# quziyan/NPairLoss

Measured on NVIDIA H100. Metric: N-pair fwd+bwd samples/sec at B=8192,D=512, higher is better.
Workload: dtype f32 (3-pass fp16-split wgmma, f32 accumulate)

## Files before the change

### npairloss_b200/csrc/ctx.cu

```cuda
#include <cuda.h>
#include <cuda_bf16.h>
#include <cuda_fp16.h>
#include <cuda_runtime.h>
#include <sched.h>
#include <cudaTypedefs.h>
#include <dlfcn.h>

#include <cstdarg>
#include <cstdio>
#include <cstdlib>
#include <cmath>
#include <cstring>
#include <map>
#include <memory>
#include <mutex>
#include <string>
#include <vector>

#include "../../include/npair_b200.h"
#include "gemm_wgmma.cuh"
#include "grad_fused.cuh"
#include "host.cuh"
#include "kernels.cuh"

// ... 14 lines not shown
  fn_ncclGetUniqueId GetUniqueId = nullptr;
  fn_ncclCommInitRank CommInitRank = nullptr;
  fn_ncclCommDestroy CommDestroy = nullptr;
  fn_ncclAllGather AllGather = nullptr;
  fn_ncclReduceScatter ReduceScatter = nullptr;
  fn_ncclGroup GroupStart = nullptr, GroupEnd = nullptr;
  fn_ncclGetErrorString GetErrorString = nullptr;
  std::string err;
};
static NcclApi* nccl_api() {
  static NcclApi api;
  static bool tried = false;
  if (tried) return &api;
  tried = true;
  const char* env = getenv("NPAIR_NCCL_LIB");
  const char* names[] = {env, "libnccl.so.2", "libnccl.so"};
  for (const char* n : names) {
    if (!n) continue;
    api.h = dlopen(n, RTLD_NOW | RTLD_GLOBAL);
    if (api.h) break;
  }
  if (!api.h) { api.err = "libnccl.so.2 not found (set NPAIR_NCCL_LIB)"; return &api; }
#define NPAIR_SYM(name) api.name = reinterpret_cast<decltype(api.name)>(dlsym(api.h, "nccl" #name)); if (!api.name) api.err = "missing symbol nccl" #name;
  NPAIR_SYM(GetUniqueId) NPAIR_SYM(CommInitRank) NPAIR_SYM(CommDestroy) NPAIR_SYM(AllGather) NPAIR_SYM(ReduceScatter)
  NPAIR_SYM(GroupStart) NPAIR_SYM(GroupEnd) NPAIR_SYM(GetErrorString)
#undef NPAIR_SYM
  return &api;
}
enum { NCCL_FLOAT32 = 7, NCCL_SUM = 0 };

struct SharedComm { void* comm; int refs; };
static std::mutex g_comm_mu;
static std::map<std::string, SharedComm> g_comms;
static int acquire_comm(const void* id128, int world, int rank, void** out, std::string* err) {
  NcclApi* api = nccl_api();
  const std::string key(static_cast<const char*>(id128), 128);
  std::lock_guard<std::mutex> lk(g_comm_mu);
  auto it = g_comms.find(key);
  if (it != g_comms.end()) { ++it->second.refs; *out = it->second.comm; return 0; }
  NcclId id; memcpy(&id, id128, 128);
  void* comm = nullptr;
  const int r = api->CommInitRank(&comm, world, id, rank);
  if (r != 0) { *err = fmt("ncclCommInitRank: %s", api->GetErrorString(r)); return r; }
  g_comms[key] = SharedComm{comm, 1};
  *out = comm;
  return 0;
}
static void release_comm(void* comm) {
  NcclApi* api = nccl_api();
  std::lock_guard<std::mutex> lk(g_comm_mu);
  for (auto it = g_comms.begin(); it != g_comms.end(); ++it)
    if (it->second.comm == comm) {
      if (--it->second.refs == 0) { if (api->CommDestroy) api->CommDestroy(comm); g_comms.erase(it); }
      return;
    }
}

static PFN_cuTensorMapEncodeTiled_v12000 tmap_encode_fn() {
  static PFN_cuTensorMapEncodeTiled_v12000 fn = nullptr;
  if (!fn) {
    void* p = nullptr;
    cudaDriverEntryPointQueryResult qres;
    if (cudaGetDriverEntryPoint("cuTensorMapEncodeTiled", &p, cudaEnableDefault, &qres) == cudaSuccess && qres == cudaDriverEntryPointSuccess)
      fn = reinterpret_cast<PFN_cuTensorMapEncodeTiled_v12000>(p);
  }
  return fn;
}

bool make_tmap_pieces(CUtensorMap* m, const void* base, int cols, int rows, int pieces, long long ld_elems,
                      long long piece_stride_elems, int bk, int box_rows, std::string* err) {
  auto fn = tmap_encode_fn();
  if (!fn) { *err = "cuTensorMapEncodeTiled entry point not available"; return false; }
  cuuint64_t dims[3] = {static_cast<cuuint64_t>(cols), static_cast<cuuint64_t>(rows), static_cast<cuuint64_t>(pieces)};
  cuuint64_t strides[2] = {static_cast<cuuint64_t>(ld_elems) * 2ull, static_cast<cuuint64_t>(piece_stride_elems) * 2ull};
  cuuint32_t box[3] = {static_cast<cuuint32_t>(bk), static_cast<cuuint32_t>(box_rows), 1u};
  cuuint32_t estr[3] = {1u, 1u, 1u};
  const CUtensorMapSwizzle sw = (bk * 2 == 128) ? CU_TENSOR_MAP_SWIZZLE_128B : CU_TENSOR_MAP_SWIZZLE_64B;
  CUresult r = fn(m, CU_TENSOR_MAP_DATA_TYPE_UINT16, 3, const_cast<void*>(base), dims, strides, box, estr,
                  CU_TENSOR_MAP_INTERLEAVE_NONE, sw, CU_TENSOR_MAP_L2_PROMOTION_L2_256B, CU_TENSOR_MAP_FLOAT_OOB_FILL_NONE);
  if (r != CUDA_SUCCESS) { *err = fmt("cuTensorMapEncodeTiled failed (%d): cols=%d rows=%d pieces=%d ld=%lld", (int)r, cols, rows, pieces, ld_elems); return false; }
  return true;
}

bool make_tmap_kcat(CUtensorMap* a, CUtensorMap* b, const uint16_t* A, int rows_a, const uint16_t* B, int rows_b, long long kcat,
                    std::string* err) {
  return make_tmap_pieces(a, A, static_cast<int>(kcat), rows_a, 1, kcat, rows_a * kcat, 64, 128, err) &&
         make_tmap_pieces(b, B, static_cast<int>(kcat), rows_b, 1, kcat, rows_b * kcat, 64, 256, err);
}

bool make_tmap_f32_store(CUtensorMap* m, const void* base, int cols, int rows, long long ld_elems, std::string* err, int box_rows) {
  auto fn = tmap_encode_fn();
  if (!fn) { *err = "cuTensorMapEncodeTiled entry point not available"; return false; }
  cuuint64_t dims[2] = {static_cast<cuuint64_t>(cols), static_cast<cuuint64_t>(rows)};
  cuuint64_t strides[1] = {static_cast<cuuint64_t>(ld_elems) * 4ull};
  cuuint32_t box[2] = {32u, static_cast<cuuint32_t>(box_rows)};
  cuuint32_t estr[2] = {1u, 1u};
  CUresult r = fn(m, CU_TENSOR_MAP_DATA_TYPE_FLOAT32, 2, const_cast<void*>(base), dims, strides, box, estr,
                  CU_TENSOR_MAP_INTERLEAVE_NONE, CU_TENSOR_MAP_SWIZZLE_128B, CU_TENSOR_MAP_L2_PROMOTION_NONE, CU_TENSOR_MAP_FLOAT_OOB_FILL_NONE);
  if (r != CUDA_SUCCESS) { *err = fmt("cuTensorMapEncodeTiled(S) failed (%d): cols=%d rows=%d ld=%lld", (int)r, cols, rows, ld_elems); return false; }
  return true;
}

__global__ void p2p_push_kernel(const float* __restrict__ srcA, long long nA, long long offA, const float* __restrict__ srcB, long long nB, long long offB,
                                float* const* __restrict__ peer_base, long long flags_off , int flag_index, int world, uint32_t epoch,
                                unsigned int* ticket) {
  const long long tid = static_cast<long long>(blockIdx.x) * blockDim.x + threadIdx.x, nth = static_cast<long long>(gridDim.x) * blockDim.x;
  const bool vecA = (nA & 3) == 0 && (offA & 3) == 0 && (reinterpret_cast<uintptr_t>(srcA) & 15) == 0;
  if (vecA) {
    for (long long i = tid; i < (nA >> 2); i += nth) {
      const float4 v = reinterpret_cast<const float4*>(srcA)[i];
      for (int r = 0; r < world; ++r) reinterpret_cast<float4*>(peer_base[r] + offA)[i] = v;
    }
  } else {
    for (long long i = tid; i < nA; i += nth) { const float v = srcA[i]; for (int r = 0; r < world; ++r) peer_base[r][offA + i] = v; }
  }
  for (long long i = tid; i < nB; i += nth) { const float v = srcB[i]; for (int r = 0; r < world; ++r) peer_base[r][offB + i] = v; }
  __threadfence_system();
  __syncthreads();
  __shared__ int s_last;
  if (threadIdx.x == 0) s_last = (atomicAdd(ticket, 1u) == gridDim.x - 1) ? 1 : 0;
  __syncthreads();
  if (!s_last) return;
  __threadfence_system();
  if (static_cast<int>(threadIdx.x) < world) {
    uint32_t* f = reinterpret_cast<uint32_t*>(peer_base[threadIdx.x] + flags_off) + flag_index;
    asm volatile("st.release.sys.global.u32 [%0], %1;" ::"l"(f), "r"(epoch) : "memory");
  }
  if (threadIdx.x == 0) *ticket = 0;
}
__global__ void p2p_wait_kernel(const uint32_t* __restrict__ flags , int world, uint32_t epoch) {
  if (static_cast<int>(threadIdx.x) < world) {
    uint32_t v;
    do { asm volatile("ld.acquire.sys.global.u32 %0, [%1];" : "=r"(v) : "l"(flags + threadIdx.x) : "memory"); } while (static_cast<int32_t>(v - epoch) < 0);
  }
}

}

using namespace npair;

#define NPAIR_PROF_PHASES 9
#define NPAIR_INTERNAL_FULL_TILES (1 << 30)
#define NPAIR_XCH_FLOATS 8192
#define NPAIR_H100_SXM_SMS 132

enum { XP_X, XP_LAB, XP_REC, XP_XCH, XP_COUNT };
struct XchgLayout {
  long long base[XP_COUNT], par_stride[XP_COUNT], rank_stride[XP_COUNT], flags, floats;
  long long off(int part, long long par, int rank) const { return base[part] + par * par_stride[part] + rank * rank_stride[part]; }
};
static XchgLayout xchg_layout(int Q, int D, int world, bool world_scope) {
  const long long N = static_cast<long long>(Q) * world;
  const long long rank_floats[XP_COUNT] = {static_cast<long long>(Q) * D, Q, ROW_RECORD_FLOATS * Q, world_scope ? NPAIR_XCH_FLOATS : 0};
  const long long par_floats[XP_COUNT] = {N * D, round_up(N, 4), ROW_RECORD_FLOATS * N, world * rank_floats[XP_XCH]};
  XchgLayout l;
  long long o = 0;
  for (int p = 0; p < XP_COUNT; ++p) { l.base[p] = o; l.par_stride[p] = par_floats[p]; l.rank_stride[p] = rank_floats[p]; o += 2 * par_floats[p]; }
  l.flags = o;
  l.floats = o + round_up(6ll * world, 4);
  return l;
}
static_assert(NPAIR_XCH_FLOATS % 2 == 0, "XCH slots hold 64-bit fields");
enum { XCHG_FEATURES, XCHG_RECORDS, XCHG_SMALL };
static inline int xchg_flag(int kind, int par, int world, int rank) { return (2 * kind + par) * world + rank; }

static int sim_block_rows(const npair_config& c) {
  const long long h = 128ll * ((c.flags >> NPAIR_SIM_BLOCK_SHIFT) & 0xFFF);
  return h < c.Q ? static_cast<int>(h) : 0;
}

static int select_mask(const npair_config& c, int region) {
  return (c.ap_region == region && is_rel(c.ap_method) && !sn_is_max(c.identsn) ? 1 : 0) |
         (c.an_region == region && is_rel(c.an_method) && !sn_is_max(c.diffsn) ? 2 : 0);
}

struct Plan {
  int N, nsplit, bk_grad;
  long long Dp, Np, Qp, ldS;
  long long kcat;
  int bwd_mode;
  bool fused_grad;
  bool cat;
  unsigned int gcand_cap;
  int grad_chunk_kb;
  int grad_kblocks;
  SplitK grad_split;
  int split_cap;
  int n_sym_tiles;
  int s_rows;
  int n_blocks;
  int sweep_epi;
  bool wscope;
  int lsel_mask, gsel_mask;
  bool want_p2p_feat, want_p2p_rec;
  XchgLayout xl;
};

static Plan plan_of(const npair_config& cfg, int sms, bool mma_symmetric, int mem_rows = 0) {
  Plan p{};
  const int prec = cfg.sim_precision, W = cfg.world;
  const long long Q = cfg.Q, D = cfg.D, N = Q * W + mem_rows;
  const bool tc = cfg.gemm_backend == NPAIR_GEMM_TCGEN05, multi = W > 1;
  p.N = static_cast<int>(N);
  p.nsplit = SPLIT_FORMATS[prec].pieces; p.bk_grad = bk_of(prec, EPI_OUT);
  p.Dp = round_up(D, 64); p.Np = round_up(N, 64); p.Qp = round_up(Q, 64); p.ldS = round_up(N, 32);
  p.kcat = mma_passes(p.nsplit) * p.Dp;
  const int blk_rows = sim_block_rows(cfg);
  p.s_rows = blk_rows ? blk_rows : cfg.Q;
  p.n_blocks = (cfg.Q + p.s_rows - 1) / p.s_rows;
  p.wscope = cfg.global_scope && multi;
  p.lsel_mask = select_mask(cfg, NPAIR_LOCAL);
  p.gsel_mask = select_mask(cfg, NPAIR_GLOBAL);
  p.bwd_mode = !multi ? NPAIR_BWDMODE_SINGLE
             : (cfg.bwd_exchange == NPAIR_BWD_AUTO && (!tc || mma_symmetric)) ? NPAIR_BWDMODE_ROW_SCALARS : NPAIR_BWDMODE_REDUCE_SCATTER;
  const bool rs = p.bwd_mode == NPAIR_BWDMODE_REDUCE_SCATTER;
  p.fused_grad = tc && !rs && !(cfg.flags & NPAIR_FLAG_NO_FUSED_GRAD);
  p.cat = tc && prec != PREC_BF16;
  if (p.gsel_mask) {
    const long long cap = Q * N / 8 + 4096;
    p.gcand_cap = static_cast<unsigned int>(cap < (32ll << 20) ? cap : (32ll << 20));
  }
  p.grad_chunk_kb = cfg.grad_chunk_cols > 0 ? (cfg.grad_chunk_cols + 31) / 32 : (cfg.grad_chunk_cols < 0 ? 0 : 64);
  p.grad_kblocks = static_cast<int>(p.fused_grad ? (N + 31) / 32 : (N + p.bk_grad - 1) / p.bk_grad);
  const int tiles = tile_sched(cfg.Q, cfg.D, p.grad_kblocks).num_tiles();
  p.grad_split = tc ? split_k(p.grad_kblocks, tiles, sms, p.fused_grad ? 8 : 4) : SplitK{1, p.grad_kblocks};
  p.split_cap = tc ? split_k_cap(p.grad_kblocks, tiles, sms, p.fused_grad ? 8 : 4) : 1;
  if (!multi && tc && !(cfg.flags & NPAIR_INTERNAL_FULL_TILES) && mem_rows == 0) p.n_sym_tiles = static_cast<int>(sym_tile_count(cfg.Q, p.N));
  p.sweep_epi = EPI_STATS | (p.n_sym_tiles ? EPI_SYM : 0) | (p.n_blocks == 1 ? EPI_STORE_S : 0);
  p.want_p2p_feat = multi && W <= 32 && !(cfg.flags & NPAIR_FLAG_NCCL_FEATURES);
  p.want_p2p_rec = multi && W <= 32 && !(cfg.flags & NPAIR_FLAG_NCCL_RECORDS) && p.bwd_mode == NPAIR_BWDMODE_ROW_SCALARS;
  if (p.want_p2p_feat || p.want_p2p_rec) p.xl = xchg_layout(cfg.Q, cfg.D, W, p.wscope);
  return p;
}

static void carve_rows(Carve& cv, long long Q, long long mem_cap, RowArrays* ra) {
  carve_stats(cv, Q, ra);
  ra->posi_thr = cv.take<float>(Q); ra->nega_thr = cv.take<float>(Q);
  ra->A = cv.take<float>(Q); ra->T = cv.take<float>(Q); ra->logv = cv.take<float>(Q);
  ra->hits = cv.take<int>(3 * Q);
  ra->rowrec = cv.take<RowRecord>(Q + mem_cap, 32);
}

struct npair_ctx : Plan {
  npair_config cfg;
  int Q, D, world, rank, prec, sms, device;
  int mem_cap = 0;
  int mem_rows = 0;
  float* labcat = nullptr;
  DevMem mem;
  float* Xtot_buf = nullptr;
  float* labtot_buf = nullptr;
  float* S = nullptr;
  uint16_t *Xs = nullptr, *XsT = nullptr, *XlT = nullptr, *H = nullptr, *HT = nullptr;
  float* OUT2 = nullptr;
  uint16_t *XcatA = nullptr, *XcatB = nullptr;
  RowRecord* rs_total = nullptr;
  float *Ynorm = nullptr, *dY = nullptr, *inv_norm = nullptr;
  CUtensorMap tm_fB, tm_fS;
  bool p2p_feat = false, p2p_rec = false;
  float* p2p_region = nullptr;
  uint32_t xch_epoch = 0;
  float* xch_src = nullptr;
  float* xch_all = nullptr;
  float** p2p_peer_base = nullptr;
  unsigned int* p2p_ticket = nullptr;
  std::vector<void*> p2p_opened;
  uint32_t p2p_fwd_epoch = 0, p2p_rec_epoch = 0;
  int2* sym_tiles = nullptr;
  int s_block_row0 = -1;
  float* part = nullptr;
  RowArrays ra;
  BlockScalars* bs = nullptr;
  float* partial = nullptr;
  unsigned long long* ghist = nullptr;
  uint32_t* gcand = nullptr;
  TopsBlock* tops_pinned = nullptr;
  unsigned int tops_seq = 0;
  TopsBlock* tops_dev = nullptr;
  AsyncWords* aw = nullptr;
  struct Capture { cudaStream_t st = nullptr; unsigned long long id = 0; } capture;
  CUtensorMap tm_simA, tm_simB, tm_S, tm_b1A, tm_b1B, tm_b2A, tm_b2B;
  void* comm = nullptr; bool own_comm = false;
  struct Step {
    const float* label = nullptr;
    const float *x_total = nullptr, *lab_total = nullptr;
    bool ext_gathered = false;
    bool rec_gathered = false;
    bool fwd_done = false;
    const float *x_mem = nullptr, *lab_mem = nullptr;
  } step;
  StreamOrder order;
  std::string err;
  bool prof = false;
  cudaEvent_t ev[NPAIR_PROF_PHASES + 1][2];
  bool ev_made = false;
  bool ev_used[NPAIR_PROF_PHASES] = {};
};

static cudaError_t ctx_buffers(npair_ctx* c, DevMem& m) {
  const long long Q = c->cfg.Q, D = c->cfg.D, N = c->N;
  const size_t f = sizeof(float), ns = c->nsplit;
  if (c->mem_cap) m.own(&c->labcat, f * N, false);
  if (c->cfg.world > 1) { m.own(&c->Xtot_buf, f * N * D, false); m.own(&c->labtot_buf, f * N, false); }
  if (c->cfg.normalize_input) { m.own(&c->Ynorm, f * Q * D, false); m.own(&c->dY, f * Q * D, false); m.own(&c->inv_norm, f * Q, false); }
  m.own(&c->S, f * c->s_rows * c->ldS, true);
  if (!c->cat) m.own(&c->Xs, 2 * ns * N * c->Dp, true);
  m.own(&c->XsT, 2 * ns * D * c->Np, true);
  if (c->cat) { m.own(&c->XcatA, 2 * Q * c->cfg.world * c->kcat, true); m.own(&c->XcatB, 2 * N * c->kcat, true); }
  if (!c->fused_grad) m.own(&c->H, 2 * ns * Q * c->Np, true);
  if (c->bwd_mode == NPAIR_BWDMODE_REDUCE_SCATTER) { m.own(&c->XlT, 2 * ns * D * c->Qp, true); m.own(&c->HT, 2 * ns * N * c->Qp, true); m.own(&c->OUT2, f * N * D, false); }
  if (c->bwd_mode == NPAIR_BWDMODE_ROW_SCALARS) m.own(&c->rs_total, sizeof(RowRecord) * N, false);
  const int slices = c->mem_cap ? c->split_cap : c->grad_split.splits;
  if (slices > 1) m.own(&c->part, f * split_part(slices, c->cfg.Q, D), false);
  m.own_carved(true, [c](Carve& cv) { carve_rows(cv, c->cfg.Q, c->mem_cap, &c->ra); });
  m.own(&c->bs, sizeof(BlockScalars), true);
  m.own(&c->aw, sizeof(AsyncWords), true);
  m.own(&c->partial, f * 2048, false);
  m.own(&c->ghist, sizeof(unsigned long long) * 4096, true);
  m.own(&c->gcand, sizeof(uint32_t) * 2ull * c->gcand_cap, false);
  m.own(&c->sym_tiles, sizeof(int2) * (c->mem_cap ? sym_tile_count(c->cfg.Q, c->cfg.Q) : c->n_sym_tiles), false);
  if (c->wscope) { m.own(&c->xch_src, f * NPAIR_XCH_FLOATS, false); m.own(&c->xch_all, f * NPAIR_XCH_FLOATS * c->cfg.world, false); }
  return m.err;
}
static cudaError_t p2p_buffers(npair_ctx* c, DevMem& m) {
  m.own(&c->p2p_region, sizeof(float) * c->xl.floats, true);
  m.own(&c->p2p_ticket, sizeof(unsigned int), true);
  m.own(&c->p2p_peer_base, sizeof(float*) * c->cfg.world, false);
  return m.err;
}

struct PhaseTimer {
  npair_ctx* c; int ph; cudaStream_t st;
  PhaseTimer(npair_ctx* c_, int ph_, cudaStream_t st_) : c(c_), ph(ph_), st(st_) {
    if (c->prof) { cudaEventRecord(c->ev[ph][0], st); }
  }
  ~PhaseTimer() {
    if (c->prof) { cudaEventRecord(c->ev[ph][1], st); c->ev_used[ph] = true; }
  }
};

int npair::open_device(int device, int* dev, int* sms) {
  int ndev = 0;
  if (cudaGetDeviceCount(&ndev) != cudaSuccess || ndev < 1) {
    g_create_err = "no CUDA device: libnpair_b200 has no CPU fallback (the oracle under oracle/ is test-only)";
    return NPAIR_E_CUDA;
  }
  if (device >= 0) CREATE_TRY(cudaSetDevice(device));
  CREATE_TRY(cudaGetDevice(dev));
  cudaDeviceProp prop;
  CREATE_TRY(cudaGetDeviceProperties(&prop, *dev));
  if (prop.major != 9 || prop.minor != 0) {
    g_create_err = fmt("device %d is sm_%d%d; this library contains sm_90a code only", *dev, prop.major, prop.minor);
    return NPAIR_E_CUDA;
  }
  *sms = prop.multiProcessorCount;
  return NPAIR_OK;
}

static int validate(const npair_config* c, std::string* err) {
  if (!c) { *err = "null config"; return NPAIR_E_ARG; }
  if (c->Q < 1 || c->D < 1) { *err = "Q and D must be >= 1"; return NPAIR_E_ARG; }
  if (c->world < 1 || c->rank < 0 || c->rank >= c->world) { *err = "bad world/rank"; return NPAIR_E_ARG; }
  if (c->num_tops < 1 || c->num_tops > 5) { *err = "num_tops must be 1..5 (npair_multi_class_loss.hpp:32-34)"; return NPAIR_E_ARG; }
  if (c->ap_region < 0 || c->ap_region > 1 || c->an_region < 0 || c->an_region > 1) { *err = "bad mining region"; return NPAIR_E_ARG; }
  if (c->ap_method < 0 || c->ap_method > 4 || c->an_method < 0 || c->an_method > 4) { *err = "bad mining method"; return NPAIR_E_ARG; }
  if (c->sim_precision < 0 || c->sim_precision > 2) { *err = "bad sim_precision"; return NPAIR_E_ARG; }
  if (c->gemm_backend < 0 || c->gemm_backend > 1) { *err = "bad gemm_backend"; return NPAIR_E_ARG; }
  if (c->bwd_exchange < 0 || c->bwd_exchange > 1) { *err = "bad bwd_exchange"; return NPAIR_E_ARG; }
  if (static_cast<long long>(c->Q) * c->world > 0x7fffffffLL) { *err = "N = Q*world exceeds int32"; return NPAIR_E_ARG; }
  if (c->global_scope < 0 || c->global_scope > 1 || c->normalize_input < 0 || c->normalize_input > 1) { *err = "global_scope / normalize_input must be 0 or 1"; return NPAIR_E_ARG; }
  if (c->grad_chunk_cols > 0 && (c->grad_chunk_cols & 31)) { *err = "grad_chunk_cols must be a multiple of 32"; return NPAIR_E_ARG; }
  if (c->global_scope && c->world > 1 && (c->bwd_exchange != NPAIR_BWD_AUTO || c->gemm_backend != NPAIR_GEMM_TCGEN05 || (c->flags & NPAIR_FLAG_NO_FUSED_GRAD))) {
    *err = "global_scope needs the row-record backward (bwd_exchange AUTO, tensor-core backend, fused gradient kernel)"; return NPAIR_E_ARG;
  }
  if (sim_block_rows(*c)) {
    if (c->gemm_backend != NPAIR_GEMM_TCGEN05 || (c->flags & NPAIR_FLAG_NO_FUSED_GRAD) || c->bwd_exchange != NPAIR_BWD_AUTO) {
      *err = "row-block similarity mode needs the tensor-core backend, the fused gradient kernel and bwd_exchange AUTO"; return NPAIR_E_ARG;
    }
    if (c->global_scope) { *err = "row-block similarity mode does not support global_scope"; return NPAIR_E_ARG; }
    if (select_mask(*c, NPAIR_GLOBAL)) {
      *err = "row-block similarity mode: a GLOBAL RELATIVE_* side needs SN >= 0 with floor(SN) = 0 (its general-SN select sweeps the whole block)";
      return NPAIR_E_ARG;
    }
  }
  return NPAIR_OK;
}

static int validate_memory(const npair_config* c, long long M, std::string* err) {
  if (M < 0) { *err = "max_memory_rows must be >= 0"; return NPAIR_E_ARG; }
  if (M == 0) return NPAIR_OK;
  if (c->world != 1) { *err = "a cross-batch memory needs world = 1"; return NPAIR_E_ARG; }
// ... 22 lines not shown
  std::string e;
  if (validate(cfg, &e) != NPAIR_OK || validate_memory(cfg, max_memory_rows, &e) != NPAIR_OK) return 0;
  npair_ctx c;
  c.cfg = *cfg;
  c.mem_cap = max_memory_rows;
  static_cast<Plan&>(c) = plan_of(*cfg, NPAIR_H100_SXM_SMS, true, max_memory_rows);
  DevMem sizing(false);
  ctx_buffers(&c, sizing);
  if (c.want_p2p_feat || c.want_p2p_rec) p2p_buffers(&c, sizing);
  return sizing.bytes;
}
size_t npair_workspace_bytes(const npair_config* cfg) { return npair_memory_workspace_bytes(cfg, 0); }

const char* npair_last_error(const npair_ctx* ctx) { return ctx ? ctx->err.c_str() : g_create_err.c_str(); }

int npair_nccl_unique_id(void* out) {
  if (!out) return NPAIR_E_ARG;
  NcclApi* api = nccl_api();
  if (!api->h || !api->err.empty()) { g_create_err = api->err; return NPAIR_E_NCCL; }
  NcclId id;
  int r = api->GetUniqueId(&id);
  if (r != 0) { g_create_err = fmt("ncclGetUniqueId: %s", api->GetErrorString(r)); return NPAIR_E_NCCL; }
  memcpy(out, &id, 128);
  return NPAIR_OK;
}

void npair_destroy(npair_ctx* c) {
  if (!c) return;
  if (c->device >= 0) cudaSetDevice(c->device);
  for (void* q : c->p2p_opened) cudaIpcCloseMemHandle(q);
  c->mem.release();
  if (c->comm && c->own_comm) release_comm(c->comm);
  if (c->tops_pinned) cudaFreeHost(c->tops_pinned);
  if (c->ev_made) for (int i = 0; i < NPAIR_PROF_PHASES; ++i) { cudaEventDestroy(c->ev[i][0]); cudaEventDestroy(c->ev[i][1]); }
  delete c;
}

static int create_impl(const npair_config* cfg, const void* id128, void* ext_comm, int mem_cap, npair_ctx** out);
static bool mma_is_symmetric(int prec, int device) {
  static std::mutex mu;
  static std::map<std::pair<int, int>, bool> cache;
  std::lock_guard<std::mutex> lk(mu);
  const std::pair<int, int> key(device, prec);
  auto it = cache.find(key);
  if (it != cache.end()) return it->second;
  bool ok = false;
  const int Q = 192, D = 96;
  npair_config cfg;
  npair_config_default(&cfg, Q, D);
  cfg.sim_precision = prec; cfg.device = device; cfg.flags = NPAIR_INTERNAL_FULL_TILES; cfg.num_tops = 2;
  npair_ctx* t = nullptr;
  if (create_impl(&cfg, nullptr, nullptr, 0, &t) == NPAIR_OK) {
    std::vector<float> x(static_cast<size_t>(Q) * D), lab(Q), S(static_cast<size_t>(Q) * t->ldS);
    uint32_t rng = 12345u;
    for (int r = 0; r < Q; ++r) {
      double nrm = 0.0;
      for (int d = 0; d < D; ++d) { rng = rng * 1664525u + 1013904223u; const float v = static_cast<float>(static_cast<int32_t>(rng >> 8) % 2001 - 1000) * 1e-3f; x[static_cast<size_t>(r) * D + d] = v; nrm += static_cast<double>(v) * v; }
      const float inv = static_cast<float>(1.0 / sqrt(nrm > 0 ? nrm : 1.0));
      for (int d = 0; d < D; ++d) x[static_cast<size_t>(r) * D + d] *= inv;
      lab[r] = static_cast<float>(r / 2);
    }
    float *dx = nullptr, *dl = nullptr;
    float tops[5];
    if (cudaMalloc(&dx, sizeof(float) * x.size()) == cudaSuccess && cudaMalloc(&dl, sizeof(float) * Q) == cudaSuccess &&
        cudaMemcpy(dx, x.data(), sizeof(float) * x.size(), cudaMemcpyHostToDevice) == cudaSuccess &&
        cudaMemcpy(dl, lab.data(), sizeof(float) * Q, cudaMemcpyHostToDevice) == cudaSuccess &&
        npair_forward(t, dx, dl, tops, nullptr) == NPAIR_OK && cudaDeviceSynchronize() == cudaSuccess &&
        cudaMemcpy(S.data(), t->S, sizeof(float) * S.size(), cudaMemcpyDeviceToHost) == cudaSuccess) {
      ok = true;
      for (int i = 0; i < Q && ok; ++i)
        for (int j = 0; j < i; ++j)
          if (memcmp(&S[static_cast<size_t>(i) * t->ldS + j], &S[static_cast<size_t>(j) * t->ldS + i], 4) != 0) { ok = false; break; }
    }
    cudaFree(dx); cudaFree(dl);
    npair_destroy(t);
  }
  cudaGetLastError();
  cache[key] = ok;
  return ok;
}

static bool make_maps(npair_ctx* c, std::string* te) {
  const int Q = c->Q, D = c->D, N = c->N, ns = c->nsplit, bkg = c->bk_grad;
  const uint16_t* catA = c->cat ? c->XcatA : c->Xs;
  const uint16_t* catB = c->cat ? c->XcatB : c->Xs;
  bool ok = make_tmap_kcat(&c->tm_simA, &c->tm_simB, catA +static_cast<long long>(c->rank) * Q * c->kcat, Q, catB, N, c->kcat, te);
  ok = ok && make_tmap_f32_store(&c->tm_S, c->S, N, c->s_rows, c->ldS, te);
  if (c->H) ok = ok && make_tmap_pieces(&c->tm_b1A, c->H, N, Q, ns, c->Np, static_cast<long long>(Q) * c->Np, bkg, 128, te);
  ok = ok && make_tmap_pieces(&c->tm_b1B, c->XsT, N, D, ns, c->Np, static_cast<long long>(D) * c->Np, bkg, 256, te);
  if (c->fused_grad) {
    ok = ok && make_tmap_pieces(&c->tm_fB, c->XsT, N, D, ns, c->Np, static_cast<long long>(D) * c->Np, 32, 256, te);
    ok = ok && make_tmap_f32_store(&c->tm_fS, c->S, N, c->s_rows, c->ldS, te, 128);
  }
  if (c->bwd_mode == NPAIR_BWDMODE_REDUCE_SCATTER) {
    ok = ok && make_tmap_pieces(&c->tm_b2A, c->HT, Q, N, ns, c->Qp, static_cast<long long>(N) * c->Qp, bkg, 128, te);
    ok = ok && make_tmap_pieces(&c->tm_b2B, c->XlT, Q, D, ns, c->Qp, static_cast<long long>(D) * c->Qp, bkg, 256, te);
  }
  return ok;
}

static int set_call_rows(npair_ctx* c, int m) {
  if (!c->mem_cap || m == c->mem_rows) return NPAIR_OK;
  c->step.fwd_done = false;
  const Plan p = plan_of(c->cfg, c->sms, true, m);
  if (p.grad_split.splits > c->split_cap) {
    c->err = fmt("internal: m = %d needs %d split-K slices, the buffer holds %d", m, p.grad_split.splits, c->split_cap);
    return NPAIR_E_STATE;
  }
  c->N = p.N; c->gcand_cap = p.gcand_cap; c->grad_kblocks = p.grad_kblocks; c->grad_split = p.grad_split;
  c->n_sym_tiles = p.n_sym_tiles; c->sweep_epi = p.sweep_epi;
  c->mem_rows = -1;
  std::string te;
  if (!make_maps(c, &te)) { c->err = te; return NPAIR_E_CUDA; }
  c->mem_rows = m;
  return NPAIR_OK;
}

static int create_impl(const npair_config* cfg, const void* id128, void* ext_comm, int mem_cap, npair_ctx** out) {
  if (!out) { g_create_err = "null out"; return NPAIR_E_ARG; }
  *out = nullptr;
  std::string e;
  int rc = validate(cfg, &e);
  if (rc == NPAIR_OK) rc = validate_memory(cfg, mem_cap, &e);
  if (rc != NPAIR_OK) { g_create_err = e; return rc; }
  int device = -1, sms = 0;
  if ((rc = open_device(cfg->device, &device, &sms)) != NPAIR_OK) return rc;
  std::unique_ptr<npair_ctx, void (*)(npair_ctx*)> made(new npair_ctx(), npair_destroy);
  npair_ctx* c = made.get();
  c->cfg = *cfg; c->device = device; c->sms = sms; c->mem_cap = mem_cap; c->mem_rows = mem_cap;
  const bool blocks = sim_block_rows(*cfg) > 0;
  const bool ask_sym = (cfg->world > 1 && cfg->bwd_exchange == NPAIR_BWD_AUTO && cfg->gemm_backend == NPAIR_GEMM_TCGEN05) || blocks;
  const bool sym = !ask_sym || mma_is_symmetric(cfg->sim_precision, c->device);
  if (blocks && !sym) {
    g_create_err = "row-block similarity mode: the similarity GEMM is not bitwise symmetric on this device, so a recomputed block of S "
                   "would not match the rows the statistics were taken from";
    return NPAIR_E_ARG;
  }
  static_cast<Plan&>(*c) = plan_of(*cfg, c->sms, sym, mem_cap);
  c->Q = cfg->Q; c->D = cfg->D; c->world = cfg->world; c->rank = cfg->rank; c->prec = cfg->sim_precision;
  const int Q = c->Q;
  CREATE_TRY(ctx_buffers(c, c->mem));
  if (c->sym_tiles) {
    const std::vector<int2> tl = sym_tile_list(Q, Q);
    CREATE_TRY(cudaMemcpy(c->sym_tiles, tl.data(), sizeof(int2) * tl.size(), cudaMemcpyHostToDevice));
  }
  CREATE_TRY(cudaHostAlloc(&c->tops_pinned, sizeof(TopsBlock), cudaHostAllocMapped));
  memset(c->tops_pinned, 0, sizeof(TopsBlock));
  CREATE_TRY(cudaHostGetDevicePointer(&c->tops_dev, c->tops_pinned, 0));
  CREATE_TRY(c->order.create());
  if (c->lsel_mask) CREATE_TRY(allow_local_select_smem());
  if (cfg->gemm_backend == NPAIR_GEMM_TCGEN05) {
    CREATE_TRY(allow_smem(gemm_kernel(c->prec, c->sweep_epi)));
    if (mem_cap) CREATE_TRY(allow_smem(gemm_kernel(c->prec, plan_of(*cfg, c->sms, sym).sweep_epi)));
    if (c->n_blocks > 1) CREATE_TRY(allow_smem(gemm_kernel(c->prec, EPI_STORE_S)));
    CREATE_TRY(c->fused_grad ? allow_smem(fused_kernel(c->prec)) : allow_smem(gemm_kernel(c->prec, EPI_OUT)));
    std::string te;
    if (!make_maps(c, &te)) { g_create_err = te; return NPAIR_E_CUDA; }
  }
  if (c->world > 1 && (id128 || ext_comm)) {
    NcclApi* api = nccl_api();
    if (!api->h || !api->err.empty()) { g_create_err = api->err; return NPAIR_E_NCCL; }
    if (ext_comm) { c->comm = ext_comm; c->own_comm = false; }
    else {
      std::string ce;
      if (acquire_comm(id128, c->world, c->rank, &c->comm, &ce) != 0) { g_create_err = ce; c->comm = nullptr; return NPAIR_E_NCCL; }
      c->own_comm = true;
    }
  }
  if (c->comm && (c->want_p2p_feat || c->want_p2p_rec) && !getenv("NPAIR_NO_P2P")) {
// ... 190 lines not shown
  if ((rc = async_entry(c, stream, "npair_forward_async", &captured)) != NPAIR_OK) return rc;
  OrderedCall call(c, stream, captured);
  if ((rc = call.enter()) != NPAIR_OK) return rc;
  if ((rc = forward_rank(c, d_feat, d_label, &c->aw->tops, call.st)) != NPAIR_OK) return rc;
  return finish_forward_async(c, d_tops, call.st);
}

int npair_forward_gathered(npair_ctx* c, const float* d_feat_total, const float* d_label_total, float tops_host[5], void* stream) {
  if (!c) return NPAIR_E_ARG;
  if (!d_feat_total || !d_label_total || !tops_host) { c->err = "null pointer argument"; return NPAIR_E_ARG; }
  int rc;
  if ((rc = refuse_capture(c, stream, "npair_forward_gathered")) != NPAIR_OK) return rc;
  OrderedCall call(c, stream);
  if ((rc = call.enter()) != NPAIR_OK) return rc;
  if ((rc = set_call_rows(c, 0)) != NPAIR_OK) return rc;
  const long long r0 = static_cast<long long>(c->rank) * c->Q;
  float* const normed = c->world > 1 ? c->Xtot_buf : c->Ynorm;
  c->step = npair_ctx::Step{d_label_total + r0, c->cfg.normalize_input ? normed : d_feat_total, d_label_total, true};
  if (c->cfg.normalize_input) {
    PhaseTimer pt(c, 1, call.st);
    launch_l2norm_fwd(d_feat_total, c->N, c->D, normed, nullptr, call.st);
    launch_l2norm_fwd(d_feat_total + r0 * c->D, c->Q, c->D, c->Ynorm, c->inv_norm, call.st);
  }
  if ((rc = forward_impl(c, c->step.x_total + r0 * c->D, c->tops_dev, call.st)) != NPAIR_OK) return rc;
  return finish_forward(c, tops_host, call.st);
}

static int memory_call_args(npair_ctx* c, int m) {
  const int rc = validate_memory(&c->cfg, 1, &c->err);
  if (rc != NPAIR_OK) return rc;
  if (m < 0 || m > c->mem_cap) { c->err = fmt("m = %d memory rows outside [0, %d] (npair_create_memory)", m, c->mem_cap); return NPAIR_E_ARG; }
  return NPAIR_OK;
}
static int forward_memory_rows(npair_ctx* c, const float* d_feat, const float* d_label, const float* d_mem_feat, const float* d_mem_label, int m,
                               TopsBlock* tops, cudaStream_t st) {
  const int rc = set_call_rows(c, m);
  if (rc != NPAIR_OK) return rc;
  c->step = npair_ctx::Step{d_label, nullptr, c->labcat};
  c->step.x_mem = d_mem_feat; c->step.lab_mem = d_mem_label;
  if (c->cfg.normalize_input) {
    PhaseTimer pt(c, 1, st);
    launch_l2norm_fwd(d_feat, c->Q, c->D, c->Ynorm, c->inv_norm, st);
    d_feat = c->Ynorm;
  }
  c->step.x_total = d_feat;
  return forward_impl(c, d_feat, tops, st);
}

int npair_forward_memory(npair_ctx* c, const float* d_feat, const float* d_label, const float* d_mem_feat, const float* d_mem_label, int32_t m,
                         float tops_host[5], void* stream) {
  if (!c) return NPAIR_E_ARG;
  if (!d_feat || !d_label || !tops_host || (m > 0 && (!d_mem_feat || !d_mem_label))) { c->err = "null pointer argument"; return NPAIR_E_ARG; }
  int rc;
  if ((rc = memory_call_args(c, m)) != NPAIR_OK) return rc;
  if (m == 0) return npair_forward(c, d_feat, d_label, tops_host, stream);
  if ((rc = refuse_capture(c, stream, "npair_forward_memory")) != NPAIR_OK) return rc;
  OrderedCall call(c, stream);
  if ((rc = call.enter()) != NPAIR_OK) return rc;
  if ((rc = forward_memory_rows(c, d_feat, d_label, d_mem_feat, d_mem_label, m, c->tops_dev, call.st)) != NPAIR_OK) return rc;
  return finish_forward(c, tops_host, call.st);
}

int npair_forward_memory_async(npair_ctx* c, const float* d_feat, const float* d_label, const float* d_mem_feat, const float* d_mem_label,
                               int32_t m, float* d_tops, void* stream) {
  if (!c) return NPAIR_E_ARG;
  if (!d_feat || !d_label || !d_tops || (m > 0 && (!d_mem_feat || !d_mem_label))) { c->err = "null pointer argument"; return NPAIR_E_ARG; }
  int rc;
  if ((rc = memory_call_args(c, m)) != NPAIR_OK) return rc;
  if (m == 0) return npair_forward_async(c, d_feat, d_label, d_tops, stream);
  bool captured = false;
  if ((rc = async_entry(c, stream, "npair_forward_memory_async", &captured)) != NPAIR_OK) return rc;
  OrderedCall call(c, stream, captured);
  if ((rc = call.enter()) != NPAIR_OK) return rc;
  if ((rc = forward_memory_rows(c, d_feat, d_label, d_mem_feat, d_mem_label, m, &c->aw->tops, call.st)) != NPAIR_OK) return rc;
  return finish_forward_async(c, d_tops, call.st);
}

static SimRows sim_rows(const npair_ctx* c, int r0, int rows) {
  return SimRows{c->S, c->ldS, c->Q, c->N, r0, rows, c->step.label, c->step.lab_total, c->rank * c->Q};
}

static cudaError_t sim_gemm(npair_ctx* c, int epi, int r0, int rows, cudaStream_t st) {
  const SimRows sim = sim_rows(c, r0, rows);
  GemmParams gp = sim_sweep(epi, rows, c->N, c->kcat, &c->bs->x_inv_scale, c->sym_tiles, c->n_sym_tiles, c->ra);
  gp.a_row0 = sim.row0; gp.S = c->S; gp.ldS = sim.ldS;
  if (epi & EPI_STATS) {
    gp.lab_rows = sim.lab_rows; gp.lab_cols = sim.lab_cols; gp.self_offset = sim.col0;
    gp.fuse_thr = 1; gp.ra = c->ra; gp.mp = mining_of(c->cfg); gp.bs = c->bs;
    gp.thr_out = c->wscope ? reinterpret_cast<BlockStats*>(c->xch_src) : nullptr;
  }
  return launch_gemm(c->prec, epi, c->tm_simA, c->tm_simB, c->tm_S, gp, c->sms, st);
}

static cudaError_t recompute_sim_block(npair_ctx* c, int r0, cudaStream_t st) {
  if (c->s_block_row0 == r0) return cudaSuccess;
  const cudaError_t e = sim_gemm(c, EPI_STORE_S, r0, c->Q - r0 < c->s_rows ? c->Q - r0 : c->s_rows, st);
  c->s_block_row0 = e == cudaSuccess ? r0 : -1;
  return e;
}

static int forward_impl(npair_ctx* c, const float* d_feat, TopsBlock* tops, cudaStream_t st) {
  const int Q = c->Q, N = c->N, D = c->D;
  const MiningParams mp = mining_of(c->cfg);
  const int self_off = c->rank * Q;
  const bool lsel_warp = (c->cfg.flags & NPAIR_FLAG_LSEL_WARP) != 0;
  {
    PhaseTimer pt(c, 1, st);
    if (c->step.x_mem) {
      const int m = N - Q;
      launch_memory_rows(c->step.label, Q, c->step.lab_mem, m, c->labcat, c->ra.rowrec, st);
      launch_prep_reduce_memory(d_feat, static_cast<long long>(Q) * D, c->step.x_mem, static_cast<long long>(m) * D, c->partial,
                                c->prec == PREC_FP16X2 ? 1 : 0, c->ra, Q, c->bs, st);
      launch_split_memory(d_feat, Q, c->step.x_mem, N, D, c->prec, c->bs, c->Xs, c->Dp, c->XsT, c->Np, c->XcatA, c->XcatB, c->Dp, st);
    } else {
      launch_prep_reduce(d_feat, static_cast<long long>(Q) * D, c->step.x_total, static_cast<long long>(N) * D, c->partial,
                         c->prec == PREC_FP16X2 ? 1 : 0, c->ra, Q, c->bs, st);
      launch_split(c->step.x_total, N, D, c->prec, c->bs, c->Xs, c->Dp, c->XsT, c->Np, c->XlT, c->Qp, self_off, Q, c->XcatA, c->XcatB, c->Dp, st);
    }
  }
  c->s_block_row0 = c->n_blocks == 1 ? 0 : -1;
  if (c->cfg.gemm_backend == NPAIR_GEMM_TCGEN05) {
    PhaseTimer pt(c, 2, st);
    CUDA_TRY(c, sim_gemm(c, c->sweep_epi, 0, Q, st));
  } else {
    GemmParams gp; memset(&gp, 0, sizeof(gp));
    gp.M = Q; gp.Nn = N; gp.S = c->S; gp.ldS = c->ldS; gp.dev_scale = &c->bs->x_inv_scale;
    CUDA_TRY(c, launch_simt_gemm(c->prec, EPI_STORE_S, c->Xs + static_cast<long long>(self_off) * c->Dp, c->Dp, static_cast<long long>(N) * c->Dp,
                                 c->Xs, c->Dp, static_cast<long long>(N) * c->Dp, D, gp, st));
    launch_row_stats_ref(sim_rows(c, 0, Q), c->ra, st);
  }
  {
    PhaseTimer pt(c, 3, st);
    if (c->cfg.gemm_backend != NPAIR_GEMM_TCGEN05) launch_thresholds(c->ra, Q, N, mp, c->bs, st);
    if (c->wscope) {
      const float* all = nullptr;
      const int rc = xchg_small(c, c->xch_src, sizeof(BlockStats) / sizeof(float), &all, st);
      if (rc != NPAIR_OK) return rc;
      launch_thresholds_world(all, NPAIR_XCH_FLOATS, c->world, N, mp, c->bs, st);
    }
    if (c->gsel_mask) {
      for (int pass = 0; pass < 3; ++pass) {
        launch_global_select_pass(sim_rows(c, 0, Q), c->gsel_mask, pass, c->ra, c->ghist, c->gcand, c->gcand_cap, c->wscope ? 1 : 0, c->bs, c->sms,
                                  st);
        if (c->wscope) {
          const float* all = nullptr;
          const int rc = xchg_small(c, reinterpret_cast<const float*>(c->ghist), NPAIR_XCH_FLOATS, &all, st);
          if (rc != NPAIR_OK) return rc;
          launch_global_decide(all, NPAIR_XCH_FLOATS, c->world, c->gsel_mask, pass, c->ra, Q, c->ghist, c->gcand, c->gcand_cap, c->bs, st);
        }
      }
    }
    if (c->lsel_mask && c->n_blocks == 1)
      launch_local_select(sim_rows(c, 0, Q), c->lsel_mask, c->cfg.identsn, c->cfg.diffsn, c->ra, c->bs, c->sms, lsel_warp, st);
  }
  {
    PhaseTimer pt(c, 4, st);
    ++c->tops_seq;
    for (int r0 = 0; r0 < Q; r0 += c->s_rows) {
      const int rows = Q - r0 < c->s_rows ? Q - r0 : c->s_rows;
      CUDA_TRY(c, recompute_sim_block(c, r0, st));
      const SimRows sim = sim_rows(c, r0, rows);
      if (c->lsel_mask && c->n_blocks > 1)
        launch_local_select(sim, c->lsel_mask, c->cfg.identsn, c->cfg.diffsn, c->ra, c->bs, c->sms, lsel_warp, st);
      launch_lse_rows(sim, mp, c->ra, c->bs, c->cfg.num_tops, tops, c->world, c->wscope ? reinterpret_cast<TopSums*>(c->xch_src) : nullptr,
                      weight_scale_log2(c->prec), c->tops_seq, c->n_blocks == 1, st);
    }
    if (c->n_blocks > 1) launch_lse_finalize(Q, N, c->ra, c->bs, c->cfg.num_tops, tops, c->tops_seq, st);
// ... 405 lines not shown
```

### npairloss_b200/csrc/device.cuh

```cuda
#pragma once
#include <cuda_bf16.h>
#include <cuda_fp16.h>
#include <cfloat>

#include "kernels.cuh"

namespace npair {

__device__ __forceinline__ float warp_sum(float v) {
#pragma unroll
  for (int o = 16; o > 0; o >>= 1) v += __shfl_xor_sync(0xffffffffu, v, o);
  return v;
}
__device__ __forceinline__ int warp_sum_i(int v) {
#pragma unroll
  for (int o = 16; o > 0; o >>= 1) v += __shfl_xor_sync(0xffffffffu, v, o);
  return v;
}
__device__ __forceinline__ float warp_max(float v) {
#pragma unroll
  for (int o = 16; o > 0; o >>= 1) v = fmaxf(v, __shfl_xor_sync(0xffffffffu, v, o));
  return v;
}
__device__ __forceinline__ float warp_min(float v) {
#pragma unroll
  for (int o = 16; o > 0; o >>= 1) v = fminf(v, __shfl_xor_sync(0xffffffffu, v, o));
  return v;
}

template <int PREC>
__device__ __forceinline__ void split3(float v, uint16_t& p0, uint16_t& p1, uint16_t& p2) {
  if (PREC == PREC_BF16) {
    p0 = __bfloat16_as_ushort(__float2bfloat16_rn(v)); p1 = 0; p2 = 0;
  } else if (PREC == PREC_FP16X2) {
    const __half h = __float2half_rn(v);
    const float r = v - __half2float(h);
    p0 = __half_as_ushort(h); p1 = __half_as_ushort(__float2half_rn(r)); p2 = 0;
  } else {
    const __nv_bfloat16 h = __float2bfloat16_rn(v);
    const float r1 = v - __bfloat162float(h);
    const __nv_bfloat16 m = __float2bfloat16_rn(r1);
    const float r2 = r1 - __bfloat162float(m);
    p0 = __bfloat16_as_ushort(h); p1 = __bfloat16_as_ushort(m); p2 = __bfloat16_as_ushort(__float2bfloat16_rn(r2));
  }
}
template <int PREC>
__device__ __forceinline__ void split8(const float (&v)[8], float sc, uint16_t (&p)[8][3], uint4 (&pk)[3]) {
#pragma unroll
  for (int e = 0; e < 8; ++e) split3<PREC>(v[e] * sc, p[e][0], p[e][1], p[e][2]);
#pragma unroll
  for (int s = 0; s < SPLIT_FORMATS[PREC].pieces; ++s)
    pk[s] = make_uint4(p[0][s] | (static_cast<uint32_t>(p[1][s]) << 16), p[2][s] | (static_cast<uint32_t>(p[3][s]) << 16),
                       p[4][s] | (static_cast<uint32_t>(p[5][s]) << 16), p[6][s] | (static_cast<uint32_t>(p[7][s]) << 16));
}
template <int PREC>
__device__ __forceinline__ void store_kcat_row(uint16_t* row, long long Dp, int d, const uint4 (&pk)[3], bool side_b) {
  *reinterpret_cast<uint4*>(row + d) = pk[0];
  if (PREC == PREC_FP16X2) {
    *reinterpret_cast<uint4*>(row + Dp + 2 * d) = side_b ? pk[1] : pk[0];
    *reinterpret_cast<uint4*>(row + Dp + 2 * d + 8) = side_b ? pk[0] : pk[1];
  } else if (PREC == PREC_BF16X3) {
    *reinterpret_cast<uint4*>(row + Dp + d) = pk[1];
    *reinterpret_cast<uint4*>(row + 2 * Dp + 2 * d) = side_b ? pk[1] : pk[0];
    *reinterpret_cast<uint4*>(row + 2 * Dp + 2 * d + 8) = side_b ? pk[0] : pk[1];
    *reinterpret_cast<uint4*>(row + 4 * Dp + 2 * d) = side_b ? pk[2] : pk[0];
    *reinterpret_cast<uint4*>(row + 4 * Dp + 2 * d + 8) = side_b ? pk[0] : pk[2];
  }
}

__device__ __forceinline__ void reset_row_stats(const RowArrays& ra, long long i) {
  ra.st_minw[i] = f2ord(FLT_MAX); ra.st_maxw[i] = f2ord(-FLT_MAX);
  ra.st_maxb[i] = f2ord(-FLT_MAX); ra.st_maxall[i] = f2ord(-FLT_MAX);
  ra.cnt_same[i] = 0;
}

}
```

### npairloss_b200/csrc/eval.cu

```cuda
#include <cuda_runtime.h>

#include <cmath>
#include <cstdint>
#include <memory>
#include <string>
#include <vector>

#include "../../include/npair_b200.h"
#include "gemm_wgmma.cuh"
#include "host.cuh"
#include "kernels.cuh"

using namespace npair;

static constexpr int EVAL_NO_SELF = -(1 << 30);

struct EvalPlan {
  int max_q, max_g, D, prec;
  long long Dp, kcat;
  int n_sym_tiles;
};

static int eval_validate(long long max_q, long long max_g, long long D, int prec, std::string* err) {
  if (max_q < 1 || max_g < 1 || D < 1) { *err = "max_queries, max_gallery and D must be >= 1"; return NPAIR_E_ARG; }
  if (max_q >= (1 << 30) || max_g >= (1 << 30) || D >= (1 << 24)) { *err = "max_queries and max_gallery must be < 2^30, D < 2^24"; return NPAIR_E_ARG; }
  if (prec < 0 || prec > 2) { *err = "bad precision"; return NPAIR_E_ARG; }
  return NPAIR_OK;
}

static EvalPlan eval_plan_of(int max_q, int max_g, int D, int prec) {
  EvalPlan p{};
  p.max_q = max_q; p.max_g = max_g; p.D = D; p.prec = prec;
  p.Dp = round_up(D, 64);
  p.kcat = mma_passes(SPLIT_FORMATS[prec].pieces) * p.Dp;
  const int n = max_q < max_g ? max_q : max_g;
  p.n_sym_tiles = static_cast<int>(sym_tile_count(n, n));
  return p;
}

struct npair_eval : EvalPlan {
  int device = -1, sms = 0;
  DevMem mem;
  uint16_t *catA = nullptr, *catB = nullptr;
  RowArrays ra{};
  unsigned int* absmax_bits = nullptr;
  BlockScalars* bs = nullptr;
  int2* sym_tiles = nullptr;
  int sym_n = 0;
  std::vector<int2> sym_host;
  DevMem map_rows_mem, map_pairs_mem, km_mem, knn_mem, cb_mem;
  char *map_rows = nullptr, *map_pairs = nullptr, *km = nullptr, *knn = nullptr, *cb = nullptr;
  StreamOrder order;
  std::string err;
};

static cudaError_t eval_buffers(npair_eval* ev, DevMem& m) {
  m.own(&ev->catA, 2ull * ev->max_q * ev->kcat, false);
  m.own(&ev->catB, 2ull * ev->max_g * ev->kcat, false);
  m.own_carved(true, [ev](Carve& cv) { carve_stats(cv, ev->max_q, &ev->ra); ev->absmax_bits = cv.take<unsigned int>(1); });
  m.own(&ev->bs, sizeof(BlockScalars), true);
  m.own(&ev->sym_tiles, sizeof(int2) * ev->n_sym_tiles, false);
  return m.err;
}

struct MapRows : Carve {
  long long* seg; unsigned long long* sum_err; int* fill;
  MapRows(char* base, long long nq) : Carve{base} { seg = take<long long>(nq + 1); sum_err = take<unsigned long long>(2); fill = take<int>(nq); }
};
struct MapPairs : Carve {
  float* pos; unsigned int* hist;
  MapPairs(char* base, long long sum_r) : Carve{base} { pos = take<float>(sum_r); hist = take<unsigned int>(sum_r); }
};
struct KmeansBufs : Carve {
  long long* sums; unsigned long long* keys; double* partial; int* counts; float* bias; int* rows; KmeansWords* words;
  KmeansBufs(char* base, long long n, long long k, long long D) : Carve{base} {
    sums = take<long long>(k * D); keys = take<unsigned long long>(n); partial = take<double>(KM_INERTIA_BLOCKS);
    counts = take<int>(k); bias = take<float>(k); rows = take<int>(k); words = take<KmeansWords>(1);
  }
};
struct KnnBlock : Carve {
  float* S; long long ldS;
  KnnBlock(char* base, long long rows, long long ng) : Carve{base}, ldS(round_up(ng, 32)) { S = take<float>(rows * ldS); }
};
static_assert(KNN_MAX_K == NPAIR_EVAL_KNN_MAX_K, "the select's capacity is the call's limit on k");
static constexpr int KNN_DEFAULT_BLOCK_ROWS = 1024;
static int knn_block_rows(int block_rows, int nq) {
  const long long rows = block_rows ? block_rows : KNN_DEFAULT_BLOCK_ROWS, cap = round_up(nq, 128);
  return static_cast<int>(rows < cap ? rows : cap);
}
struct ClassBatchBufs : Carve {
  float* S; long long ldS; int* pools;
  ClassBatchBufs(char* base, long long C, long long pool_size, long long n_batches) : Carve{base}, ldS(round_up(C, 32)) {
    S = take<float>(C * ldS); pools = take<int>(n_batches * pool_size);
  }
};
static_assert(CLASS_POOL_MAX == NPAIR_EVAL_CLASS_POOL_MAX, "the greedy kernel's capacity is the call's limit on the pool size");

static int eval_grow(npair_eval* ev, DevMem& m, char** base, size_t bytes, const char* what) {
  if (bytes <= m.bytes) return NPAIR_OK;
  m.release();
  m.own(base, bytes, false);
  if (m.err == cudaSuccess) return NPAIR_OK;
  cudaGetLastError();
  m.release();
  ev->err = fmt("cannot allocate %zu bytes for %s", bytes, what);
  return NPAIR_E_CUDA;
}

extern "C" {

size_t npair_eval_workspace_bytes(int32_t max_q, int32_t max_g, int32_t D, int32_t prec) {
  std::string e;
  if (eval_validate(max_q, max_g, D, prec, &e) != NPAIR_OK) return 0;
  npair_eval ev;
  static_cast<EvalPlan&>(ev) = eval_plan_of(max_q, max_g, D, prec);
  DevMem sizing(false);
  eval_buffers(&ev, sizing);
  return sizing.bytes;
}

size_t npair_eval_map_at_r_bytes(int32_t nq, int64_t sum_r) {
  if (nq < 1 || sum_r < 0) return 0;
  return MapRows(nullptr, nq).bytes + MapPairs(nullptr, sum_r).bytes;
}

size_t npair_eval_kmeans_bytes(int32_t n, int32_t k, int32_t D) {
  if (n < 1 || k < 1 || D < 1 || k > n) return 0;
  return KmeansBufs(nullptr, n, k, D).bytes;
}

size_t npair_eval_knn_bytes(int32_t ng, int32_t k, int32_t block_rows) {
  if (ng < 1 || k < 1 || k > NPAIR_EVAL_KNN_MAX_K || k > ng || block_rows < 0 || block_rows % 128) return 0;
  return KnnBlock(nullptr, block_rows ? block_rows : KNN_DEFAULT_BLOCK_ROWS, ng).bytes;
}

size_t npair_eval_class_batches_bytes(int32_t n_classes, int32_t pool_size, int32_t n_batches) {
  if (n_classes < 1 || n_batches < 1 || pool_size < 2 || pool_size > n_classes || pool_size > NPAIR_EVAL_CLASS_POOL_MAX) return 0;
  return ClassBatchBufs(nullptr, n_classes, pool_size, n_batches).bytes;
}

const char* npair_eval_last_error(const npair_eval* ev) { return ev ? ev->err.c_str() : g_create_err.c_str(); }

void npair_eval_destroy(npair_eval* ev) {
  if (!ev) return;
  if (ev->device >= 0) cudaSetDevice(ev->device);
  delete ev;
}

int npair_eval_create(int32_t max_q, int32_t max_g, int32_t D, int32_t prec, int32_t device, npair_eval** out) {
  if (!out) { g_create_err = "null out"; return NPAIR_E_ARG; }
  *out = nullptr;
  int rc = eval_validate(max_q, max_g, D, prec, &g_create_err);
  if (rc != NPAIR_OK) return rc;
  int dev = -1, sms = 0;
  if ((rc = open_device(device, &dev, &sms)) != NPAIR_OK) return rc;
  std::unique_ptr<npair_eval, void (*)(npair_eval*)> made(new npair_eval(), npair_eval_destroy);
  npair_eval* ev = made.get();
  static_cast<EvalPlan&>(*ev) = eval_plan_of(max_q, max_g, D, prec);
  ev->device = dev; ev->sms = sms;
  CREATE_TRY(eval_buffers(ev, ev->mem));
  CREATE_TRY(ev->order.create());
  const int epis[] = {EPI_STATS, EPI_STATS | EPI_SYM, EPI_COUNT, EPI_COUNT | EPI_SYM, EPI_GATHER, EPI_GATHER | EPI_SYM, EPI_BUCKET,
                      EPI_BUCKET | EPI_SYM, EPI_ARGMAX, EPI_STORE_S};
  for (int epi : epis) CREATE_TRY(allow_smem(gemm_kernel(prec, epi)));
  CREATE_TRY(allow_knn_select_smem());
  *out = made.release();
  return NPAIR_OK;
}

}

static int eval_check(npair_eval* ev, const float* q, int nq, const float* g, int ng, int self_offset, int gallery_row0, float absmax,
                      bool whole_gallery) {
  if (!q || !g) { ev->err = "null pointer argument"; return NPAIR_E_ARG; }
  if (nq < 1 || ng < 1) { ev->err = "nq and ng must be >= 1"; return NPAIR_E_ARG; }
  if (nq > ev->max_q || ng > ev->max_g) { ev->err = fmt("nq = %d, ng = %d exceed the evaluator's capacity (%d, %d)", nq, ng, ev->max_q, ev->max_g); return NPAIR_E_ARG; }
  if (self_offset < -1) { ev->err = "self_offset must be -1 (disjoint sets) or >= 0"; return NPAIR_E_ARG; }
  if (whole_gallery && self_offset >= 0 && static_cast<long long>(self_offset) + nq > ng) { ev->err = "self_offset + nq exceeds ng"; return NPAIR_E_ARG; }
  if (gallery_row0 < 0) { ev->err = "gallery_row0 must be >= 0"; return NPAIR_E_ARG; }
  if (!(absmax >= 0.f) && !whole_gallery) { ev->err = "absmax must be max|x| over the queries and the whole gallery (>= 0)"; return NPAIR_E_ARG; }
  if (!std::isfinite(absmax) && !whole_gallery) { ev->err = "absmax must be finite"; return NPAIR_E_ARG; }
  return NPAIR_OK;
}

static int eval_self_col(int self_offset, int gallery_row0) { return self_offset < 0 ? EVAL_NO_SELF : self_offset - gallery_row0; }
static bool eval_sym(const float* q, int nq, const float* g, int ng, int self_col) { return q == g && nq == ng && self_col == 0; }

static int eval_prepare(npair_eval* ev, const float* q, int nq, const float* g, int ng, float absmax, bool sym, cudaStream_t st) {
  const long long D = ev->D;
  unsigned int* amx = nullptr;
  if (absmax < 0.f && ev->prec == PREC_FP16X2) {
    amx = ev->absmax_bits;
    CUDA_TRY(ev, cudaMemsetAsync(amx, 0, sizeof(unsigned int), st));
  }
  launch_eval_prep(q, nq * D, sym ? nullptr : g, ng * D, amx, ev->ra, nq, ev->sms, st);
  launch_eval_split(q, nq, ev->D, ev->Dp, ev->prec, 0, absmax, amx, ev->bs, ev->catA, st);
  launch_eval_split(g, ng, ev->D, ev->Dp, ev->prec, 1, absmax, amx, ev->bs, ev->catB, st);
  CUDA_TRY(ev, cudaGetLastError());
  return NPAIR_OK;
}

static int eval_sweep(npair_eval* ev, int epi, int nq, int ng, int self_col, const float* ql, const float* gl, const float* cut, int32_t* count,
                      bool sym, cudaStream_t st, const GemmParams* map = nullptr) {
  if (sym) {
    if (ev->sym_n != nq) {
      ev->sym_host = sym_tile_list(nq, nq);
      CUDA_TRY(ev, cudaMemcpyAsync(ev->sym_tiles, ev->sym_host.data(), sizeof(int2) * ev->sym_host.size(), cudaMemcpyHostToDevice, st));
      ev->sym_n = nq;
    }
    epi |= EPI_SYM;
  }
  GemmParams gp = sim_sweep(epi, nq, ng, ev->kcat, &ev->bs->x_inv_scale, ev->sym_tiles, static_cast<int>(ev->sym_host.size()), ev->ra);
  gp.self_offset = self_col;
  if (epi & (EPI_STATS | EPI_GATHER | EPI_BUCKET)) { gp.lab_rows = ql; gp.lab_cols = gl; }
  else { gp.cut = cut; gp.count = count; }
  if (map) {
    gp.cnt_same = ev->ra.cnt_same; gp.bs = ev->bs; gp.seg = map->seg; gp.fill = map->fill; gp.pos = map->pos; gp.hist = map->hist;
    gp.col_bias = map->col_bias; gp.best = map->best;
  }
  CUtensorMap ta, tb;
  std::string te;
  if (!make_tmap_kcat(&ta, &tb, ev->catA, nq, ev->catB, ng, ev->kcat, &te)) { ev->err = te; return NPAIR_E_CUDA; }
  CUDA_TRY(ev, launch_gemm(ev->prec, epi, ta, tb, ta, gp, ev->sms, st));
  return NPAIR_OK;
}

extern "C" {

int npair_eval_rank(npair_eval* ev, const float* q, const float* ql, int32_t nq, const float* g, const float* gl, int32_t ng, int32_t self_offset,
                    int32_t* d_rank, void* stream) {
  if (!ev) return NPAIR_E_ARG;
  int rc = eval_check(ev, q, nq, g, ng, self_offset, 0, -1.f, true);
  if (rc != NPAIR_OK) return rc;
  if (!ql || !gl || !d_rank) { ev->err = "null pointer argument"; return NPAIR_E_ARG; }
  OrderedCall call(ev, stream);
  if ((rc = call.enter()) != NPAIR_OK) return rc;
  const cudaStream_t st = call.st;
  const int self_col = eval_self_col(self_offset, 0);
  const bool sym = eval_sym(q, nq, g, ng, self_col);
  float* cut = reinterpret_cast<float*>(ev->ra.st_minw);
  if ((rc = eval_prepare(ev, q, nq, g, ng, -1.f, sym, st)) != NPAIR_OK) return rc;
  if ((rc = eval_sweep(ev, EPI_STATS, nq, ng, self_col, ql, gl, nullptr, nullptr, sym, st)) != NPAIR_OK) return rc;
  launch_eval_best(ev->ra, nq, cut, st);
  CUDA_TRY(ev, cudaMemsetAsync(d_rank, 0, sizeof(int32_t) * nq, st));
  if ((rc = eval_sweep(ev, EPI_COUNT, nq, ng, self_col, nullptr, nullptr, cut, d_rank, sym, st)) != NPAIR_OK) return rc;
  CUDA_TRY(ev, cudaGetLastError());
  return NPAIR_OK;
}

int npair_eval_best_positive(npair_eval* ev, const float* q, const float* ql, int32_t nq, const float* g, const float* gl, int32_t ng,
                             int32_t self_offset, int32_t gallery_row0, float absmax, float* d_best, void* stream) {
  if (!ev) return NPAIR_E_ARG;
  int rc = eval_check(ev, q, nq, g, ng, self_offset, gallery_row0, absmax, false);
  if (rc != NPAIR_OK) return rc;
  if (!ql || !gl || !d_best) { ev->err = "null pointer argument"; return NPAIR_E_ARG; }
  OrderedCall call(ev, stream);
  if ((rc = call.enter()) != NPAIR_OK) return rc;
  const cudaStream_t st = call.st;
  const int self_col = eval_self_col(self_offset, gallery_row0);
  const bool sym = eval_sym(q, nq, g, ng, self_col);
  if ((rc = eval_prepare(ev, q, nq, g, ng, absmax, sym, st)) != NPAIR_OK) return rc;
  if ((rc = eval_sweep(ev, EPI_STATS, nq, ng, self_col, ql, gl, nullptr, nullptr, sym, st)) != NPAIR_OK) return rc;
  launch_eval_best(ev->ra, nq, d_best, st);
  CUDA_TRY(ev, cudaGetLastError());
  return NPAIR_OK;
}

int npair_eval_count(npair_eval* ev, const float* q, int32_t nq, const float* g, int32_t ng, int32_t self_offset, int32_t gallery_row0,
                     float absmax, const float* d_cut, int32_t* d_count, void* stream) {
  if (!ev) return NPAIR_E_ARG;
  int rc = eval_check(ev, q, nq, g, ng, self_offset, gallery_row0, absmax, false);
  if (rc != NPAIR_OK) return rc;
  if (!d_cut || !d_count) { ev->err = "null pointer argument"; return NPAIR_E_ARG; }
  OrderedCall call(ev, stream);
  if ((rc = call.enter()) != NPAIR_OK) return rc;
  const cudaStream_t st = call.st;
  const int self_col = eval_self_col(self_offset, gallery_row0);
  const bool sym = eval_sym(q, nq, g, ng, self_col);
  if ((rc = eval_prepare(ev, q, nq, g, ng, absmax, sym, st)) != NPAIR_OK) return rc;
  CUDA_TRY(ev, cudaMemsetAsync(d_count, 0, sizeof(int32_t) * nq, st));
  if ((rc = eval_sweep(ev, EPI_COUNT, nq, ng, self_col, nullptr, nullptr, d_cut, d_count, sym, st)) != NPAIR_OK) return rc;
  CUDA_TRY(ev, cudaGetLastError());
  return NPAIR_OK;
}

int npair_eval_knn(npair_eval* ev, const float* q, int32_t nq, const float* g, int32_t ng, int32_t self_offset, int32_t gallery_row0,
                   float absmax, int32_t k, int32_t block_rows, float* d_sim, int32_t* d_index, void* stream) {
  if (!ev) return NPAIR_E_ARG;
  int rc = eval_check(ev, q, nq, g, ng, self_offset, gallery_row0, absmax < 0.f ? 0.f : absmax, false);
  if (rc != NPAIR_OK) return rc;
  if (!d_sim || !d_index) { ev->err = "null pointer argument"; return NPAIR_E_ARG; }
  if (static_cast<long long>(gallery_row0) + ng > INT32_MAX) { ev->err = "gallery_row0 + ng exceeds the int32 index range"; return NPAIR_E_ARG; }
  if (block_rows < 0 || block_rows % 128) { ev->err = fmt("block_rows = %d must be 0 or a positive multiple of 128", block_rows); return NPAIR_E_ARG; }
  long long self_col = self_offset < 0 ? EVAL_NO_SELF : static_cast<long long>(self_offset) - gallery_row0;
  if (self_col >= ng || self_col + nq <= 0) self_col = EVAL_NO_SELF;
  const int valid = self_col == EVAL_NO_SELF ? ng : ng - 1;
  if (k < 1 || k > NPAIR_EVAL_KNN_MAX_K || k > valid) {
    ev->err = fmt("k = %d must lie in [1, %d] and not exceed the %d candidate columns of a query", k, NPAIR_EVAL_KNN_MAX_K, valid);
    return NPAIR_E_ARG;
  }
  OrderedCall call(ev, stream);
  if ((rc = call.enter()) != NPAIR_OK) return rc;
  const cudaStream_t st = call.st;
  const int rows = knn_block_rows(block_rows, nq);
  if ((rc = eval_grow(ev, ev->knn_mem, &ev->knn, KnnBlock(nullptr, rows, ng).bytes, "the k-NN block of S")) != NPAIR_OK) return rc;
  const KnnBlock blk(ev->knn, rows, ng);
  if ((rc = eval_prepare(ev, q, nq, g, ng, absmax, false, st)) != NPAIR_OK) return rc;
  CUtensorMap ta, tb;
  std::string te;
  if (!make_tmap_kcat(&ta, &tb, ev->catA, nq, ev->catB, ng, ev->kcat, &te)) { ev->err = te; return NPAIR_E_CUDA; }
  for (int r0 = 0; r0 < nq; r0 += rows) {
    const int m = nq - r0 < rows ? nq - r0 : rows;
    GemmParams gp = sim_sweep(EPI_STORE_S, m, ng, ev->kcat, &ev->bs->x_inv_scale, nullptr, 0, ev->ra);
    gp.a_row0 = r0; gp.S = blk.S; gp.ldS = blk.ldS;
    CUDA_TRY(ev, launch_gemm(ev->prec, EPI_STORE_S, ta, tb, ta, gp, ev->sms, st));
    launch_knn_select(blk.S, blk.ldS, m, ng, k, r0, static_cast<int>(self_col), gallery_row0, d_sim, d_index, st);
  }
  CUDA_TRY(ev, cudaGetLastError());
  return NPAIR_OK;
}

int npair_eval_class_batches(npair_eval* ev, const float* x, int32_t C, const int32_t* pools, int32_t P, int32_t nb, int32_t n,
                             int32_t* d_batches, float* d_scores, void* stream) {
  if (!ev) return NPAIR_E_ARG;
  if (!x || !pools || !d_batches) { ev->err = "null pointer argument"; return NPAIR_E_ARG; }
  if (C < 1 || C > ev->max_q || C > ev->max_g) {
    ev->err = fmt("n_classes = %d must lie in [1, %d]: the evaluator's capacity (%d, %d)", C, ev->max_q < ev->max_g ? ev->max_q : ev->max_g,
                  ev->max_q, ev->max_g);
    return NPAIR_E_ARG;
  }
  if (P < 2 || P > C || P > NPAIR_EVAL_CLASS_POOL_MAX) {
    ev->err = fmt("pool_size = %d must lie in [2, %d] (n_classes = %d, NPAIR_EVAL_CLASS_POOL_MAX = %d)", P,
                  C < NPAIR_EVAL_CLASS_POOL_MAX ? C : NPAIR_EVAL_CLASS_POOL_MAX, C, NPAIR_EVAL_CLASS_POOL_MAX);
    return NPAIR_E_ARG;
  }
  if (n < 2 || n > P) { ev->err = fmt("classes_per_batch = %d must lie in [2, pool_size = %d]", n, P); return NPAIR_E_ARG; }
  if (nb < 1) { ev->err = "n_batches must be >= 1"; return NPAIR_E_ARG; }
  std::vector<int> seen(C, -1);
  for (int t = 0; t < nb; ++t)
    for (int j = 0; j < P; ++j) {
      const int id = pools[static_cast<long long>(t) * P + j];
      if (id < 0 || id >= C) { ev->err = fmt("pool %d position %d: class %d is not in [0, %d)", t, j, id, C); return NPAIR_E_ARG; }
      if (seen[id] == t) { ev->err = fmt("pool %d holds class %d twice", t, id); return NPAIR_E_ARG; }
      seen[id] = t;
    }
  int rc;
  OrderedCall call(ev, stream);
  if ((rc = call.enter()) != NPAIR_OK) return rc;
  const cudaStream_t st = call.st;
  if ((rc = eval_grow(ev, ev->cb_mem, &ev->cb, ClassBatchBufs(nullptr, C, P, nb).bytes, "the class set's S and the pools")) != NPAIR_OK)
    return rc;
  const ClassBatchBufs cb(ev->cb, C, P, nb);
  if ((rc = eval_prepare(ev, x, C, x, C, -1.f, false, st)) != NPAIR_OK) return rc;
  CUtensorMap ta, tb;
  std::string te;
  if (!make_tmap_kcat(&ta, &tb, ev->catA, C, ev->catB, C, ev->kcat, &te)) { ev->err = te; return NPAIR_E_CUDA; }
  GemmParams gp = sim_sweep(EPI_STORE_S, C, C, ev->kcat, &ev->bs->x_inv_scale, nullptr, 0, ev->ra);
  gp.a_row0 = 0; gp.S = cb.S; gp.ldS = cb.ldS;
  CUDA_TRY(ev, launch_gemm(ev->prec, EPI_STORE_S, ta, tb, ta, gp, ev->sms, st));
  CUDA_TRY(ev, cudaMemcpyAsync(cb.pools, pools, sizeof(int32_t) * nb * P, cudaMemcpyHostToDevice, st));
  launch_class_batches(cb.S, cb.ldS, cb.pools, P, nb, n, d_batches, d_scores, ev->sms, st);
  CUDA_TRY(ev, cudaGetLastError());
  return NPAIR_OK;
}

int npair_eval_map_at_r(npair_eval* ev, const float* q, const float* ql, int32_t nq, const float* g, const float* gl, int32_t ng,
                        int32_t self_offset, double* d_map_r, double* d_r_precision, int32_t* d_R, int32_t* d_rank, void* stream) {
  if (!ev) return NPAIR_E_ARG;
  int rc = eval_check(ev, q, nq, g, ng, self_offset, 0, -1.f, true);
  if (rc != NPAIR_OK) return rc;
  if (!ql || !gl || !d_map_r || !d_r_precision) { ev->err = "null pointer argument"; return NPAIR_E_ARG; }
  OrderedCall call(ev, stream);
  if ((rc = call.enter()) != NPAIR_OK) return rc;
  const cudaStream_t st = call.st;
  const int self_col = eval_self_col(self_offset, 0);
  const bool sym = eval_sym(q, nq, g, ng, self_col);
  if ((rc = eval_grow(ev, ev->map_rows_mem, &ev->map_rows, MapRows(nullptr, nq).bytes, "the MAP@R per-query offsets")) != NPAIR_OK) return rc;
  const MapRows rows(ev->map_rows, nq);
  const int* R = ev->ra.cnt_same;
  if ((rc = eval_prepare(ev, q, nq, g, ng, -1.f, sym, st)) != NPAIR_OK) return rc;
  if ((rc = eval_sweep(ev, EPI_STATS, nq, ng, self_col, ql, gl, nullptr, nullptr, sym, st)) != NPAIR_OK) return rc;
  launch_eval_seg_scan(R, nq, rows.seg, ev->bs, rows.sum_err, st);
  unsigned long long h[2] = {0, 0};
  CUDA_TRY(ev, cudaMemcpyAsync(h, rows.sum_err, sizeof(h), cudaMemcpyDeviceToHost, st));
  CUDA_TRY(ev, cudaStreamSynchronize(st));
  if (h[1] & DERR_GATHER_SLOT) {
    ev->err = "an earlier npair_eval_map_at_r on this evaluator gathered more positives for a query than its statistics sweep counted "
              "(that query's results were NaN)";
    return NPAIR_E_CUDA;
  }
  const long long sum_r = static_cast<long long>(h[0]);
  if ((rc = eval_grow(ev, ev->map_pairs_mem, &ev->map_pairs, MapPairs(nullptr, sum_r).bytes, "the MAP@R positive pairs")) != NPAIR_OK) return rc;
  const MapPairs pairs(ev->map_pairs, sum_r);
  CUDA_TRY(ev, cudaMemsetAsync(rows.fill, 0, sizeof(int) * nq, st));
  if (sum_r > 0) {
    GemmParams mp{};
    mp.seg = rows.seg; mp.fill = rows.fill; mp.pos = reinterpret_cast<float*>(pairs.hist);
    if ((rc = eval_sweep(ev, EPI_GATHER, nq, ng, self_col, ql, gl, nullptr, nullptr, sym, st, &mp)) != NPAIR_OK) return rc;
    launch_eval_seg_sort(R, rows.seg, nq, reinterpret_cast<const float*>(pairs.hist), pairs.pos, st);
    CUDA_TRY(ev, cudaMemsetAsync(pairs.hist, 0, sizeof(unsigned int) * sum_r, st));
    mp.pos = pairs.pos; mp.hist = pairs.hist;
    if ((rc = eval_sweep(ev, EPI_BUCKET, nq, ng, self_col, ql, gl, nullptr, nullptr, sym, st, &mp)) != NPAIR_OK) return rc;
  }
  launch_eval_map_finish(R, rows.seg, rows.fill, pairs.pos, pairs.hist, nq, d_map_r, d_r_precision, d_R, d_rank, st);
  CUDA_TRY(ev, cudaGetLastError());
  return NPAIR_OK;
}

int npair_eval_kmeans(npair_eval* ev, const float* x, int32_t n, int32_t k, const int32_t* init_rows, int32_t max_iter, float* d_centroids,
                      int32_t* d_assign, double* d_inertia, int32_t stats[3], void* stream) {
  if (!ev) return NPAIR_E_ARG;
  if (!x || !init_rows || !d_centroids || !d_assign || !stats) { ev->err = "null pointer argument"; return NPAIR_E_ARG; }
  if (n < 1 || k < 1 || k > n) { ev->err = fmt("k-means needs 1 <= k <= n (n = %d, k = %d)", n, k); return NPAIR_E_ARG; }
  if (n > ev->max_q || k > ev->max_g) {
    ev->err = fmt("n = %d points, k = %d centroids exceed the evaluator's capacity (%d, %d)", n, k, ev->max_q, ev->max_g);
    return NPAIR_E_ARG;
  }
  if (max_iter < 1) { ev->err = "max_iter must be >= 1"; return NPAIR_E_ARG; }
  for (int c = 0; c < k; ++c)
    if (init_rows[c] < 0 || init_rows[c] >= n) { ev->err = fmt("init_rows[%d] = %d is not a row of x", c, init_rows[c]); return NPAIR_E_ARG; }
  int rc;
  OrderedCall call(ev, stream);
  if ((rc = call.enter()) != NPAIR_OK) return rc;
  const cudaStream_t st = call.st;
  if ((rc = eval_grow(ev, ev->km_mem, &ev->km, KmeansBufs(nullptr, n, k, ev->D).bytes, "the k-means buffers")) != NPAIR_OK) return rc;
  const long long D = ev->D;
  const KmeansBufs km(ev->km, n, k, D);
  unsigned int* amx = ev->absmax_bits;
  CUDA_TRY(ev, cudaMemcpyAsync(km.rows, init_rows, sizeof(int) * k, cudaMemcpyHostToDevice, st));
  CUDA_TRY(ev, cudaMemsetAsync(amx, 0, sizeof(unsigned int), st));
  launch_eval_prep(x, n * D, nullptr, 0, amx, ev->ra, 0, ev->sms, st);
  launch_eval_split(x, n, ev->D, ev->Dp, ev->prec, 0, -1.f, amx, ev->bs, ev->catA, st);
  launch_km_gather(x, ev->D, km.rows, k, d_centroids, st);
  CUDA_TRY(ev, cudaMemsetAsync(d_assign, 0xFF, sizeof(int32_t) * n, st));
  CUDA_TRY(ev, cudaMemsetAsync(km.keys, 0, sizeof(unsigned long long) * n, st));
  CUDA_TRY(ev, cudaMemsetAsync(km.sums, 0, sizeof(long long) * k * D, st));
  GemmParams am{};
  am.col_bias = km.bias; am.best = km.keys;
  KmeansWords h{};
  int t = 0;
// ... 25 lines not shown
```

### npairloss_b200/csrc/eval_kernels.cu

```cuda
#include <cuda.h>
#include <cfloat>

#include "device.cuh"
#include "kernels.cuh"

namespace npair {

__global__ void __launch_bounds__(256) eval_prep_kernel(const float* __restrict__ q, long long nq_el, const float* __restrict__ g, long long ng_el,
                                                        unsigned int* absmax_bits, RowArrays ra, int nq) {
  const long long stride = static_cast<long long>(gridDim.x) * blockDim.x;
  const long long t0 = static_cast<long long>(blockIdx.x) * blockDim.x + threadIdx.x;
  if (absmax_bits) {
    float mx = 0.f;
    for (long long i = t0; i < nq_el; i += stride) mx = fmaxf(mx, fabsf(__ldg(q + i)));
    if (g) for (long long i = t0; i < ng_el; i += stride) mx = fmaxf(mx, fabsf(__ldg(g + i)));
    mx = warp_max(mx);
    if ((threadIdx.x & 31) == 0 && mx > 0.f) atomicMax(absmax_bits, __float_as_uint(mx));
  }
  for (long long i = t0; i < nq; i += stride) reset_row_stats(ra, i);
}
void launch_eval_prep(const float* q, long long nq_el, const float* g, long long ng_el, unsigned int* absmax_bits, RowArrays ra, int nq,
                      int sms, cudaStream_t st) {
  const long long work = absmax_bits ? (nq_el > ng_el ? nq_el : ng_el) / 16 : nq;
  long long nb = (work + 255) / 256;
  nb = nb < 1 ? 1 : (nb > 8 * sms ? 8 * sms : nb);
  eval_prep_kernel<<<static_cast<int>(nb), 256, 0, st>>>(q, nq_el, g, ng_el, absmax_bits, ra, nq);
  count_launch();
}

template <int PREC>
__global__ void __launch_bounds__(256) eval_split_kernel(const float* __restrict__ x, int rows, int D, long long Dp, int side_b, float absmax,
                                                         const unsigned int* __restrict__ absmax_bits, BlockScalars* bs,
                                                         uint16_t* __restrict__ out) {
  constexpr int NS = SPLIT_FORMATS[PREC].pieces;
  PreScale ps{1.f, 1.f};
  if (PREC == PREC_FP16X2) ps = pre_scale(absmax >= 0.f ? absmax : __uint_as_float(*absmax_bits));
  if (blockIdx.x == 0 && threadIdx.x == 0 && !side_b) { bs->x_scale = ps.scale; bs->x_inv_scale = ps.inv; }
  const long long groups = Dp / 8, i = static_cast<long long>(blockIdx.x) * blockDim.x + threadIdx.x;
  if (i >= rows * groups) return;
  const long long n = i / groups;
  const int d = static_cast<int>(i - n * groups) * 8;
  const float* xr = x + n * D;
  float v[8];
  if (d + 7 < D && (D & 3) == 0 && (reinterpret_cast<uintptr_t>(x) & 15) == 0) {
    const float4 a4 = __ldg(reinterpret_cast<const float4*>(xr + d)), b4 = __ldg(reinterpret_cast<const float4*>(xr + d + 4));
    v[0] = a4.x; v[1] = a4.y; v[2] = a4.z; v[3] = a4.w; v[4] = b4.x; v[5] = b4.y; v[6] = b4.z; v[7] = b4.w;
  } else {
#pragma unroll
    for (int e = 0; e < 8; ++e) v[e] = d + e < D ? __ldg(xr + d + e) : 0.f;
  }
  uint16_t p[8][3];
  uint4 pk[3];
  split8<PREC>(v, ps.scale, p, pk);
  store_kcat_row<PREC>(out + n * (mma_passes(NS) * Dp), Dp, d, pk, side_b);
}
void launch_eval_split(const float* x, int rows, int D, long long Dp, int prec, int side_b, float absmax, const unsigned int* absmax_bits,
                       BlockScalars* bs, uint16_t* out, cudaStream_t st) {
  const long long work = static_cast<long long>(rows) * (Dp / 8);
  with_prec(prec, [&](auto P) {
    eval_split_kernel<P><<<static_cast<unsigned int>((work + 255) / 256), 256, 0, st>>>(x, rows, D, Dp, side_b, absmax, absmax_bits, bs, out);
  });
  count_launch();
}

__global__ void eval_best_kernel(RowArrays ra, int nq, float* __restrict__ best) {
  const int i = blockIdx.x * blockDim.x + threadIdx.x;
  if (i < nq) best[i] = ra.cnt_same[i] > 0 ? ord2f(ra.st_maxw[i]) : -INFINITY;
}
void launch_eval_best(RowArrays ra, int nq, float* best, cudaStream_t st) {
  eval_best_kernel<<<(nq + 255) / 256, 256, 0, st>>>(ra, nq, best);
  count_launch();
}

__global__ void __launch_bounds__(1024) eval_seg_scan_kernel(const int* __restrict__ cnt, int nq, long long* __restrict__ seg, BlockScalars* bs,
                                                             unsigned long long* __restrict__ sum_err) {
  __shared__ long long s_warp[32];
  const int t = threadIdx.x, lane = t & 31, w = t >> 5;
  const int per = (nq + 1023) / 1024, i0 = min(nq, t * per), i1 = min(nq, i0 + per);
  long long run = 0;
  for (int i = i0; i < i1; ++i) run += cnt[i];
  long long incl = run;
#pragma unroll
  for (int o = 1; o < 32; o <<= 1) {
    const long long y = __shfl_up_sync(0xffffffffu, incl, o);
    if (lane >= o) incl += y;
  }
  if (lane == 31) s_warp[w] = incl;
  __syncthreads();
  if (w == 0) {
    long long x = s_warp[lane], xi = x;
#pragma unroll
    for (int o = 1; o < 32; o <<= 1) {
      const long long y = __shfl_up_sync(0xffffffffu, xi, o);
      if (lane >= o) xi += y;
    }
    s_warp[lane] = xi - x;
  }
  __syncthreads();
  long long off = s_warp[w] + incl - run;
  for (int i = i0; i < i1; ++i) { seg[i] = off; off += cnt[i]; }
  if (t == 1023) {
    seg[nq] = off;
    sum_err[0] = static_cast<unsigned long long>(off);
    sum_err[1] = static_cast<unsigned long long>(bs->err);
    bs->err = 0;
  }
}
void launch_eval_seg_scan(const int* cnt, int nq, long long* seg, BlockScalars* bs, unsigned long long* sum_err, cudaStream_t st) {
  eval_seg_scan_kernel<<<1, 1024, 0, st>>>(cnt, nq, seg, bs, sum_err);
  count_launch();
}

__global__ void __launch_bounds__(256) eval_seg_sort_kernel(const int* __restrict__ cnt, const long long* __restrict__ seg, int nq,
                                                            const float* __restrict__ src, float* __restrict__ dst) {
  const int i = (blockIdx.x * blockDim.x + threadIdx.x) >> 5, lane = threadIdx.x & 31;
  if (i >= nq) return;
  const int R = cnt[i];
  const float* s = src + seg[i];
  float* d = dst + seg[i];
  for (int a = 0; a < R; a += 32) {
    const int k = a + lane;
    const uint32_t mine = k < R ? f2ord(s[k]) : 0u;
    int r = 0;
    for (int b = 0; b < R; b += 32) {
      const uint32_t other = b + lane < R ? f2ord(s[b + lane]) : 0u;
      const int n = min(32, R - b);
      for (int j = 0; j < n; ++j) {
        const uint32_t o = __shfl_sync(0xffffffffu, other, j);
        r += (o > mine || (o == mine && b + j < k)) ? 1 : 0;
      }
    }
    if (k < R) d[r] = ord2f(mine);
  }
}
void launch_eval_seg_sort(const int* cnt, const long long* seg, int nq, const float* src, float* dst, cudaStream_t st) {
  eval_seg_sort_kernel<<<(nq + 7) / 8, 256, 0, st>>>(cnt, seg, nq, src, dst);
  count_launch();
}

__global__ void __launch_bounds__(256) eval_map_finish_kernel(const int* __restrict__ cnt, const long long* __restrict__ seg,
                                                              const int* __restrict__ fill, const float* __restrict__ pos,
// ... 231 lines not shown
```

### npairloss_b200/csrc/gemm.cu

```cuda
#include <cuda_bf16.h>
#include <cuda_fp16.h>
#include <cuda_runtime.h>

#include "gemm_wgmma.cuh"
#include "grad_fused.cuh"
#include "host.cuh"
#include "kernels.cuh"

namespace npair {

static int gemm_grid(const TileSched& ts, int sms) { return ts.num_tiles() < sms ? ts.num_tiles() : sms; }

template <int NSPLIT, bool BF16, int EPI, int BK>
static GemmKernel gemm_t() {
  using Cfg = GemmCfg<NSPLIT, BK, EPI>;
  return GemmKernel{split_gemm_kernel<NSPLIT, BF16, EPI, BK>, Cfg::THREADS, Cfg::SMEM_BYTES};
}
template <bool BF16>
static GemmKernel sim_gemm_t(int epi) {
  switch (epi) {
    case EPI_STORE_S | EPI_STATS: return gemm_t<1, BF16, EPI_STORE_S | EPI_STATS, 64>();
    case EPI_STORE_S | EPI_STATS | EPI_SYM: return gemm_t<1, BF16, EPI_STORE_S | EPI_STATS | EPI_SYM, 64>();
    case EPI_STATS: return gemm_t<1, BF16, EPI_STATS, 64>();
    case EPI_STATS | EPI_SYM: return gemm_t<1, BF16, EPI_STATS | EPI_SYM, 64>();
    case EPI_STORE_S: return gemm_t<1, BF16, EPI_STORE_S, 64>();
    case EPI_COUNT: return gemm_t<1, BF16, EPI_COUNT, 64>();
    case EPI_COUNT | EPI_SYM: return gemm_t<1, BF16, EPI_COUNT | EPI_SYM, 64>();
    case EPI_GATHER: return gemm_t<1, BF16, EPI_GATHER, 64>();
    case EPI_GATHER | EPI_SYM: return gemm_t<1, BF16, EPI_GATHER | EPI_SYM, 64>();
    case EPI_BUCKET: return gemm_t<1, BF16, EPI_BUCKET, 64>();
    case EPI_BUCKET | EPI_SYM: return gemm_t<1, BF16, EPI_BUCKET | EPI_SYM, 64>();
    case EPI_ARGMAX: return gemm_t<1, BF16, EPI_ARGMAX, 64>();
    default: return GemmKernel{nullptr, 0, 0};
  }
}
GemmKernel gemm_kernel(int prec, int epi) {
  return with_prec(prec, [epi](auto P) {
    constexpr SplitFormat f = SPLIT_FORMATS[P];
    return epi != EPI_OUT ? sim_gemm_t<f.bf16>(epi) : gemm_t<f.pieces, f.bf16, EPI_OUT, bk_of(P, EPI_OUT)>();
  });
}
cudaError_t launch_gemm(int prec, int epi, const CUtensorMap& a, const CUtensorMap& b, const CUtensorMap& sm, const GemmParams& p, int sms, cudaStream_t st) {
  const GemmKernel k = gemm_kernel(prec, epi);
  if (!k.fn) return cudaErrorInvalidValue;
  k.fn<<<gemm_grid(p.ts, sms), k.threads, k.smem, st>>>(a, b, sm, p);
  count_launch();
  return cudaGetLastError();
}

FusedKernel fused_kernel(int prec) {
  return with_prec(prec, [](auto P) {
    constexpr SplitFormat f = SPLIT_FORMATS[P];
    return FusedKernel{fused_grad_kernel<f.pieces, f.bf16>, FusedCfg<f.pieces>::THREADS, FusedCfg<f.pieces>::SMEM_BYTES};
  });
}
cudaError_t launch_fused_grad(int prec, const CUtensorMap& b, const CUtensorMap& sm, const FusedGradParams& p, int sms, cudaStream_t st) {
  const FusedKernel k = fused_kernel(prec);
  k.fn<<<gemm_grid(p.ts, sms), k.threads, k.smem, st>>>(b, sm, p);
  count_launch();
  return cudaGetLastError();
}

template <int PREC>
__device__ __forceinline__ float piece_sum(const uint16_t* base, long long off, long long ps) {
  if (PREC == PREC_BF16) return __bfloat162float(__ushort_as_bfloat16(base[off]));
  if (PREC == PREC_FP16X2) return __half2float(__ushort_as_half(base[off])) + __half2float(__ushort_as_half(base[ps + off]));
  return __bfloat162float(__ushort_as_bfloat16(base[off])) + __bfloat162float(__ushort_as_bfloat16(base[ps + off])) +
         __bfloat162float(__ushort_as_bfloat16(base[2 * ps + off]));
}
template <int PREC, int OUT>
__global__ void __launch_bounds__(256) simt_gemm_kernel(const uint16_t* __restrict__ A, long long lda, long long psA,
                                                        const uint16_t* __restrict__ B, long long ldb, long long psB, int K, GemmParams p) {
  __shared__ float As[16][65], Bs[16][65];
  const int tx = threadIdx.x & 15, ty = threadIdx.x >> 4;
  const int m0 = blockIdx.y * 64, n0 = blockIdx.x * 64;
  float acc[4][4] = {};
  for (int k0 = 0; k0 < K; k0 += 16) {
    for (int e = threadIdx.x; e < 64 * 16; e += 256) {
      const int r = e >> 4, kk = e & 15;
      const int gm = m0 + r, gn = n0 + r, gk = k0 + kk;
      As[kk][r] = (gm < p.M && gk < K) ? piece_sum<PREC>(A, static_cast<long long>(gm) * lda + gk, psA) : 0.f;
      Bs[kk][r] = (gn < p.Nn && gk < K) ? piece_sum<PREC>(B, static_cast<long long>(gn) * ldb + gk, psB) : 0.f;
    }
    __syncthreads();
#pragma unroll
    for (int kk = 0; kk < 16; ++kk) {
      float a[4], b[4];
#pragma unroll
      for (int i = 0; i < 4; ++i) { a[i] = As[kk][ty * 4 + i]; b[i] = Bs[kk][tx * 4 + i]; }
#pragma unroll
      for (int i = 0; i < 4; ++i)
#pragma unroll
        for (int j = 0; j < 4; ++j) acc[i][j] = fmaf(a[i], b[j], acc[i][j]);
    }
    __syncthreads();
  }
  const float inv = p.dev_scale ? *p.dev_scale : 1.f;
  for (int i = 0; i < 4; ++i) {
    const int row = m0 + ty * 4 + i;
    if (row >= p.M) continue;
    for (int j = 0; j < 4; ++j) {
      const int col = n0 + tx * 4 + j;
      if (col >= p.Nn) continue;
      if (!OUT) p.S[static_cast<long long>(row) * p.ldS + col] = acc[i][j] * inv * inv;
      else {
        float* d = p.out + static_cast<long long>(row) * p.ldo + col;
        float o = p.alpha * inv * acc[i][j];
        if (p.beta != 0.f) o += p.beta * *d;
        *d = o;
      }
    }
  }
}
cudaError_t launch_simt_gemm(int prec, int epi, const uint16_t* A, long long lda, long long psA, const uint16_t* B, long long ldb,
                             long long psB, int K, const GemmParams& p, cudaStream_t st) {
  dim3 grid((p.Nn + 63) / 64, (p.M + 63) / 64);
  with_prec(prec, [&](auto P) {
    auto kernel = epi == EPI_OUT ? simt_gemm_kernel<P, 1> : simt_gemm_kernel<P, 0>;
    kernel<<<grid, 256, 0, st>>>(A, lda, psA, B, ldb, psB, K, p);
  });
  count_launch();
  return cudaGetLastError();
// ... 24 lines not shown
```

### npairloss_b200/csrc/gemm_wgmma.cuh

```cuda
#pragma once
#include <cuda.h>
#include <cuda_runtime.h>
#include <cfloat>
#include <stdint.h>

#include "kernels.cuh"
#include "ptx.cuh"
#include "thresholds.cuh"

namespace npair {

enum { EPI_OUT = 1, EPI_STORE_S = 8, EPI_STATS = 16, EPI_SYM = 32, EPI_COUNT = 64, EPI_GATHER = 128, EPI_BUCKET = 256, EPI_ARGMAX = 512 };

struct Tile { int m_blk, n_blk, split, kb0, kb1; };
struct TileSched {
  int num_kblocks;
  int tiles_m, tiles_n;
  const int2* tile_list;
  int num_tiles_list;
  int splits, kb_per_split;
  __host__ __device__ int num_tiles() const { return tile_list ? num_tiles_list : tiles_m * tiles_n * splits; }
  __device__ __forceinline__ Tile at(int tile) const {
    const int mn = tile / splits, split = tile - mn * splits, kb0 = split * kb_per_split;
    int m_blk = mn / tiles_n, n_blk = mn % tiles_n;
    if (tile_list) { const int2 tl = tile_list[tile]; m_blk = tl.x; n_blk = tl.y; }
    return Tile{m_blk, n_blk, split, kb0, min(num_kblocks, kb0 + kb_per_split)};
  }
};

__host__ __device__ __forceinline__ long long split_part(int split, int rows, long long ldo) { return static_cast<long long>(split) * rows * ldo; }

struct GemmParams {
  int M, Nn;
  TileSched ts;
  float* part;
  float* S;
  long long ldS;
  const float* dev_scale;
  const float* lab_rows;
  const float* lab_cols;
  int self_offset;
  uint32_t* st_minw;
  uint32_t* st_maxw;
  uint32_t* st_maxb;
  uint32_t* st_maxall;
  int* cnt_same;
  int fuse_thr;
  RowArrays ra;
  MiningParams mp;
  BlockScalars* bs;
  float* out;
  long long ldo;
  float alpha, beta;
  int a_row0;
  const float* cut;
  int* count;
  const long long* seg;
  int* fill;
  float* pos;
  unsigned int* hist;
  const float* col_bias;
  unsigned long long* best;
  BlockStats* thr_out;
};

template <int NSPLIT, int BK_, int EPI>
struct GemmCfg {
  static constexpr int BM = 128, BN = 256;
  static constexpr int BK = BK_;
  static constexpr int ROW_BYTES = BK * 2;
  static constexpr uint32_t LAYOUT = (ROW_BYTES == 128) ? 1u : 2u;
  static constexpr uint32_t SBO = 8 * ROW_BYTES;
  static constexpr int A_PIECE = BM * ROW_BYTES;
  static constexpr int B_PIECE = BN * ROW_BYTES;
  static constexpr int STAGE_BYTES = NSPLIT * (A_PIECE + B_PIECE);
  static constexpr int NPASS = mma_passes(NSPLIT);
  static constexpr int ACC_STAGE_BYTES = (EPI != EPI_OUT) ? 2 * 64 * 64 * 4 : 0;
  static constexpr int STORE_STAGE_BYTES = (EPI != EPI_OUT) ? 8 * 4096 : 0;
  static constexpr int SMEM_AUX = 2048;
  static constexpr int SMEM_MAX = 227 * 1024;
  static constexpr int STAGES_FIT = (SMEM_MAX - SMEM_AUX - 1024 - ACC_STAGE_BYTES - STORE_STAGE_BYTES) / STAGE_BYTES;
  static constexpr int STAGES = STAGES_FIT > 6 ? 6 : STAGES_FIT;
  static constexpr int SMEM_BYTES = STAGES * STAGE_BYTES + ACC_STAGE_BYTES + STORE_STAGE_BYTES + SMEM_AUX + 1024 ;
  static constexpr int THREADS = 384;
  static_assert(STAGES >= 2 && 16 * STAGES <= 192, "operand ring");
};

template <int STAGES>
struct StageRing {
  uint64_t *full, *empty;
  int stage = 0; uint32_t phase = 0;
  __device__ explicit StageRing(uint8_t* bars) : full(reinterpret_cast<uint64_t*>(bars)), empty(full + STAGES) {}
  __device__ void init() const {
    for (int s = 0; s < STAGES; ++s) { ptx::mbar_init(&full[s], 1); ptx::mbar_init(&empty[s], 8); }
    ptx::fence_mbar_init();
  }
  __device__ uint64_t* produce(uint32_t bytes) const {
    ptx::mbar_wait(&empty[stage], phase ^ 1);
    ptx::mbar_arrive_expect_tx(&full[stage], bytes);
    return &full[stage];
  }
  __device__ void wait_full() const { ptx::mbar_wait(&full[stage], phase); }
  __device__ void release(int st, int lane) const { __syncwarp(); if (lane == 0) ptx::mbar_arrive(&empty[st]); }
  __device__ void advance() { if (++stage == STAGES) { stage = 0; phase ^= 1; } }
};

__device__ __forceinline__ void pass_pieces(int nsplit, int p, int& sa, int& sb) {
  if (nsplit == 1) { sa = 0; sb = 0; return; }
  if (nsplit == 2) { sa = (p == 2) ? 1 : 0; sb = (p == 1) ? 1 : 0; return; }
  const int A[6] = {0, 0, 1, 1, 0, 2};
  const int B[6] = {0, 1, 0, 1, 2, 0};
  sa = A[p]; sb = B[p];
}

__device__ __forceinline__ bool pair_valid(bool fast, int idx, int limit, int self_idx) { return fast || (idx < limit && idx != self_idx); }
__device__ __forceinline__ bool same_label(float lab_c, float lab_i) { return lab_c == lab_i; }

__device__ __forceinline__ void stats32(const float (&v)[32], const float* __restrict__ lab, float lab_i, bool fast, int idx0,
                                        int limit, int self_idx, float& minw, float& maxw, float& maxb, int& cnt) {
  if (fast) {
    float mnw[4] = {FLT_MAX, FLT_MAX, FLT_MAX, FLT_MAX}, mxw[4] = {-FLT_MAX, -FLT_MAX, -FLT_MAX, -FLT_MAX};
    float mxb[4] = {-FLT_MAX, -FLT_MAX, -FLT_MAX, -FLT_MAX};
    int cn[4] = {0, 0, 0, 0};
#pragma unroll
    for (int q = 0; q < 8; ++q) {
      const float4 l4 = *reinterpret_cast<const float4*>(lab + 4 * q);
      const float ll[4] = {l4.x, l4.y, l4.z, l4.w};
#pragma unroll
      for (int e = 0; e < 4; ++e) {
        const float x = v[4 * q + e];
        if (ll[e] == lab_i) { mnw[e] = fminf(mnw[e], x); mxw[e] = fmaxf(mxw[e], x); ++cn[e]; }
        else mxb[e] = fmaxf(mxb[e], x);
      }
    }
    minw = fminf(minw, fminf(fminf(mnw[0], mnw[1]), fminf(mnw[2], mnw[3])));
    maxw = fmaxf(maxw, fmaxf(fmaxf(mxw[0], mxw[1]), fmaxf(mxw[2], mxw[3])));
    maxb = fmaxf(maxb, fmaxf(fmaxf(mxb[0], mxb[1]), fmaxf(mxb[2], mxb[3])));
    cnt += (cn[0] + cn[1]) + (cn[2] + cn[3]);
  } else {
#pragma unroll
    for (int c = 0; c < 32; ++c) {
      const bool valid = pair_valid(false, idx0 + c, limit, self_idx);
      const bool same = same_label(lab[c], lab_i);
      if (valid && same) { minw = fminf(minw, v[c]); maxw = fmaxf(maxw, v[c]); ++cnt; }
      if (valid && !same) maxb = fmaxf(maxb, v[c]);
    }
  }
}

__device__ __forceinline__ float max32(const float (&v)[32]) {
  float m[8];
#pragma unroll
  for (int e = 0; e < 8; ++e) m[e] = fmaxf(fmaxf(v[e], v[8 + e]), fmaxf(v[16 + e], v[24 + e]));
  return fmaxf(fmaxf(fmaxf(m[0], m[1]), fmaxf(m[2], m[3])), fmaxf(fmaxf(m[4], m[5]), fmaxf(m[6], m[7])));
}

__device__ __forceinline__ int count32(const float (&v)[32], float cut, bool fast, int idx0, int limit, int self_idx) {
  int n = 0;
  if (fast) {
#pragma unroll
    for (int c = 0; c < 32; ++c) n += (v[c] >= cut) ? 1 : 0;
  } else {
#pragma unroll
    for (int c = 0; c < 32; ++c) n += (idx0 + c < limit && idx0 + c != self_idx && v[c] >= cut) ? 1 : 0;
  }
  return n;
}
__device__ __forceinline__ float count_cut(float c) { return c == -INFINITY ? __int_as_float(0x7fffffff) : c; }

__device__ __forceinline__ uint32_t positives32(const float* __restrict__ lab, float lab_i, bool fast, int idx0, int limit, int self_idx) {
  uint32_t m = 0;
#pragma unroll
  for (int c = 0; c < 32; ++c) m |= (pair_valid(fast, idx0 + c, limit, self_idx) && same_label(lab[c], lab_i)) ? 1u << c : 0u;
  return m;
}
template <class Val>
__device__ __forceinline__ void gather_hits(uint32_t hits, Val val, int* fill, long long seg, int R, float* pos, int* err) {
  if (!hits) return;
  int slot = atomicAdd(fill, __popc(hits));
  for (; hits; hits &= hits - 1, ++slot) {
    const float s = val(__ffs(hits) - 1);
    if (slot < R) pos[seg + slot] = s;
    else atomicOr(err, DERR_GATHER_SLOT);
  }
}
__device__ __forceinline__ uint32_t negatives32(const float (&v)[32], float cut, float p1, const float* __restrict__ lab, float lab_i, bool fast,
                                                int idx0, int limit, int self_idx, uint32_t* above) {
  uint32_t m = 0, a = 0;
#pragma unroll
  for (int c = 0; c < 32; ++c) {
    const bool neg = v[c] >= cut && pair_valid(fast, idx0 + c, limit, self_idx) && !same_label(lab[c], lab_i);
    m |= neg ? 1u << c : 0u;
    a |= (neg && v[c] >= p1) ? 1u << c : 0u;
  }
  *above = a;
  return m;
}
template <class Val>
__device__ __forceinline__ void bucket_search(uint32_t cand, Val val, const float* __restrict__ p, int R, unsigned int* hist) {
  int run_b = -1;
  unsigned int run = 0;
  for (; cand; cand &= cand - 1) {
    const float s = val(__ffs(cand) - 1);
    int lo = 1, hi = R - 1;
    while (lo < hi) {
      const int mid = (lo + hi) >> 1;
      if (p[mid] > s) lo = mid + 1;
      else hi = mid;
    }
    if (lo != run_b) {
      if (run) atomicAdd(&hist[run_b], run);
      run_b = lo; run = 0;
    }
    ++run;
  }
  if (run) atomicAdd(&hist[run_b], run);
}

__device__ __forceinline__ void argmax32(const float (&v)[32], const float* __restrict__ bias, int idx0, int valid, float& best, int& col) {
#pragma unroll
  for (int c = 0; c < 32; ++c) {
    const float s = v[c] - bias[c];
    if (c < valid && s > best) { best = s; col = idx0 + c; }
  }
}

template <int NSPLIT, bool BF16, int EPI, int BK_>
__global__ void __launch_bounds__(384, 1)
split_gemm_kernel(const __grid_constant__ CUtensorMap tmapA, const __grid_constant__ CUtensorMap tmapB,
                  const __grid_constant__ CUtensorMap tmapS, const GemmParams p) {
  using Cfg = GemmCfg<NSPLIT, BK_, EPI>;
  const int worker = static_cast<int>(blockIdx.x), num_workers = static_cast<int>(gridDim.x);
  constexpr int BM = Cfg::BM, BN = Cfg::BN, BK = Cfg::BK, STAGES = Cfg::STAGES;
  constexpr bool SYM = EPI & EPI_SYM, STORE = EPI & EPI_STORE_S, STATS = EPI & EPI_STATS, COUNT = EPI & EPI_COUNT;
  constexpr bool GATHER = EPI & EPI_GATHER, BUCKET = EPI & EPI_BUCKET, ARGMAX = EPI & EPI_ARGMAX;
  constexpr bool LABELS = STATS || GATHER || BUCKET;
  static_assert(!ARGMAX || EPI == EPI_ARGMAX, "EPI_ARGMAX is used alone, with full tiles");
  extern __shared__ uint8_t smem_raw[];
  uint8_t* smem = smem_raw + ((1024u - (ptx::smem_u32(smem_raw) & 1023u)) & 1023u);
  uint8_t* acc_stage = smem + STAGES * Cfg::STAGE_BYTES;
  uint8_t* store_stage = acc_stage + Cfg::ACC_STAGE_BYTES;
  uint8_t* aux = store_stage + Cfg::STORE_STAGE_BYTES;
  float* s_lab = reinterpret_cast<float*>(aux + 256);
  float* s_labr = reinterpret_cast<float*>(aux + 256 + 1024);
  float2* s_rng = reinterpret_cast<float2*>(aux + 256 + 1024 + 512);

  const int warp = threadIdx.x >> 5, lane = threadIdx.x & 31;
  const int num_tiles = p.ts.num_tiles();
  const float inv_scale = p.dev_scale ? *p.dev_scale : 1.f;
  const float out_scale = (EPI != EPI_OUT) ? inv_scale * inv_scale : 1.f;
  const float alpha = p.alpha * inv_scale;

  if (warp == 0 && lane == 0) {
    ptx::prefetch_tmap(&tmapA);
    ptx::prefetch_tmap(&tmapB);
    if (STORE) ptx::prefetch_tmap(&tmapS);
  }
  if (warp == 1 && lane == 0) StageRing<STAGES>(aux).init();
  __syncthreads();

  if (warp < 4) {
    asm volatile("setmaxnreg.dec.sync.aligned.u32 40;");
    if (warp == 0 && lane == 0) {
      StageRing<STAGES> ring(aux);
      for (int tile = worker; tile < num_tiles; tile += num_workers) {
        const Tile t = p.ts.at(tile);
        for (int kb = t.kb0; kb < t.kb1; ++kb) {
          uint64_t* full = ring.produce(Cfg::STAGE_BYTES);
          uint8_t* st = smem + ring.stage * Cfg::STAGE_BYTES;
#pragma unroll
          for (int s = 0; s < NSPLIT; ++s) {
            ptx::tma_load_3d(st + s * Cfg::A_PIECE, &tmapA, full, kb * BK, t.m_blk * BM + (STORE && !STATS ? p.a_row0 : 0), s);
            ptx::tma_load_3d(st + NSPLIT * Cfg::A_PIECE + s * Cfg::B_PIECE, &tmapB, full, kb * BK, t.n_blk * BN, s);
          }
          ring.advance();
        }
      }
    }
    __syncwarp();
    asm volatile("bar.sync 4, 384;" ::: "memory");
    asm volatile("setmaxnreg.inc.sync.aligned.u32 168;");
  } else {
    asm volatile("setmaxnreg.inc.sync.aligned.u32 232;");
    const int cw = warp - 4;
    const int g = cw >> 2, wi = warp & 3;
    const int ew = 2 * g + (wi & 1);
    const int half = wi >> 1;
    const int et = threadIdx.x - 128;
    uint8_t* const accs = acc_stage + g * (64 * 256);
    uint8_t* const stg = store_stage + cw * 4096;
    StageRing<STAGES> ring(aux);
    for (int tile = worker; tile < num_tiles; tile += num_workers) {
      const Tile t = p.ts.at(tile);
      const int row = t.m_blk * BM + ew * 32 + lane;
      const int col_base = t.n_blk * BN;
      float lab_i = 0.f;
      if (LABELS) {
        asm volatile("bar.sync 1, 256;" ::: "memory");
        s_lab[et] = (col_base + et < p.Nn) ? p.lab_cols[col_base + et] : 0.f;
        if (row < p.M) lab_i = p.lab_rows[row];
        if (SYM && half == 0) s_labr[ew * 32 + lane] = lab_i;
        asm volatile("bar.sync 1, 256;" ::: "memory");
        {
          const float lc = s_lab[cw * 32 + lane];
          float mn = lc, mx = lc;
#pragma unroll
          for (int o = 16; o > 0; o >>= 1) { mn = fminf(mn, __shfl_xor_sync(0xffffffffu, mn, o)); mx = fmaxf(mx, __shfl_xor_sync(0xffffffffu, mx, o)); }
          if (lane == 0) s_rng[cw] = make_float2(mn, mx);
          if (SYM && cw < 4) {
            const float lr = s_labr[cw * 32 + lane];
            float rn = lr, rx = lr;
#pragma unroll
            for (int o = 16; o > 0; o >>= 1) { rn = fminf(rn, __shfl_xor_sync(0xffffffffu, rn, o)); rx = fmaxf(rx, __shfl_xor_sync(0xffffffffu, rx, o)); }
            if (lane == 0) s_rng[8 + cw] = make_float2(rn, rx);
          }
        }
        asm volatile("bar.sync 1, 256;" ::: "memory");
      }
      if constexpr (ARGMAX) {
        asm volatile("bar.sync 1, 256;" ::: "memory");
        s_lab[et] = (col_base + et < p.Nn) ? p.col_bias[col_base + et] : 0.f;
        asm volatile("bar.sync 1, 256;" ::: "memory");
      }

      float acc[128];
#pragma unroll
      for (int i = 0; i < 128; ++i) acc[i] = 0.f;
      int prev = ring.stage;
      for (int kb = t.kb0; kb < t.kb1; ++kb) {
        ring.wait_full();
        const uint32_t a0 = ptx::smem_u32(smem + ring.stage * Cfg::STAGE_BYTES) + g * 64 * Cfg::ROW_BYTES;
        const uint32_t b0 = ptx::smem_u32(smem + ring.stage * Cfg::STAGE_BYTES) + NSPLIT * Cfg::A_PIECE;
        ptx::wgmma_fence();
#pragma unroll
        for (int ps = 0; ps < Cfg::NPASS; ++ps) {
          int sa, sb;
          pass_pieces(NSPLIT, ps, sa, sb);
#pragma unroll
          for (int k4 = 0; k4 < BK / 16; ++k4) {
            const uint64_t ad = ptx::make_kmajor_desc(a0 + sa * Cfg::A_PIECE + k4 * 32, Cfg::SBO, Cfg::LAYOUT);
            const uint64_t bd = ptx::make_kmajor_desc(b0 + sb * Cfg::B_PIECE + k4 * 32, Cfg::SBO, Cfg::LAYOUT);
            ptx::wgmma_m64n256k16_ss<BF16>(acc, ad, bd, 1u);
          }
        }
        ptx::wgmma_commit();
        ptx::wgmma_wait<1>();
        if (kb != t.kb0) ring.release(prev, lane);
        prev = ring.stage;
        ring.advance();
      }
      ptx::wgmma_wait<0>();
      ptx::fence_regs(acc);
      if (t.kb1 > t.kb0) ring.release(prev, lane);

      if (EPI == EPI_OUT) {
        float* obase = p.ts.splits > 1 ? p.part + split_part(t.split, p.M, p.ldo) : p.out;
        const float beta = p.ts.splits > 1 ? 0.f : p.beta;
        const int rbase = t.m_blk * BM + g * 64 + wi * 16 + (lane >> 2);
#pragma unroll
        for (int j = 0; j < 32; ++j) {
          const int col = col_base + 8 * j + 2 * (lane & 3);
#pragma unroll
          for (int h = 0; h < 2; ++h) {
            const int r = rbase + 8 * h;
            if (r >= p.M || col >= p.Nn) continue;
            float* dst = obase + static_cast<long long>(r) * p.ldo + col;
            float o0 = alpha * acc[4 * j + 2 * h], o1 = alpha * acc[4 * j + 2 * h + 1];
            if (col + 1 < p.Nn && (p.ldo & 1) == 0) {
              if (beta != 0.f) { const float2 old = *reinterpret_cast<const float2*>(dst); o0 += beta * old.x; o1 += beta * old.y; }
              *reinterpret_cast<float2*>(dst) = make_float2(o0, o1);
            } else {
              dst[0] = (beta != 0.f) ? o0 + beta * dst[0] : o0;
              if (col + 1 < p.Nn) dst[1] = (beta != 0.f) ? o1 + beta * dst[1] : o1;
            }
          }
        }
        continue;
      }

      float minw = FLT_MAX, maxw = -FLT_MAX, maxb = -FLT_MAX, maxall = -FLT_MAX;
      int cnt = 0;
      const int self_col = row + p.self_offset;
      const int srow = (wi & 1) * 32 + lane;
      float cut_i = 0.f;
      int cnt_ge = 0;
      if (COUNT && row < p.M) cut_i = count_cut(p.cut[row]);
      long long seg_i = 0;
      int R_i = 0, above_i = 0;
      float p1_i = 0.f, pR_i = 0.f;
      if constexpr (GATHER || BUCKET) {
        if (row < p.M) { seg_i = p.seg[row]; R_i = p.cnt_same[row]; }
      }
      if constexpr (BUCKET) {
        p1_i = count_cut(R_i ? p.pos[seg_i] : -INFINITY);
        pR_i = count_cut(R_i ? p.pos[seg_i + R_i - 1] : -INFINITY);
      }
      float arg_s = -INFINITY;
      int arg_c = -1;
#pragma unroll
      for (int cp = 0; cp < 4; ++cp) {
        asm volatile("bar.sync %0, 128;" ::"r"(2 + g) : "memory");
        {
          const int c = lane & 3;
#pragma unroll
          for (int j = 0; j < 8; ++j) {
            const int q = 2 * j + (c >> 1);
#pragma unroll
            for (int h = 0; h < 2; ++h) {
              const int r = wi * 16 + (lane >> 2) + 8 * h;
              *reinterpret_cast<float2*>(accs + r * 256 + ((q ^ (r & 7)) << 4) + (c & 1) * 8) =
                  make_float2(acc[4 * (8 * cp + j) + 2 * h], acc[4 * (8 * cp + j) + 2 * h + 1]);
            }
          }
        }
        asm volatile("bar.sync %0, 128;" ::"r"(2 + g) : "memory");
        const int ch = 2 * cp + half;
        const int col0 = col_base + ch * 32;
        const int cb = col0 >> 7;
        if ((SYM && cb < t.m_blk) || col0 >= p.Nn) continue;
        float v[32];
        if (STATS || COUNT || GATHER || BUCKET || ARGMAX) {
#pragma unroll
          for (int q = 0; q < 8; ++q) {
            const float4 t4 = *reinterpret_cast<const float4*>(accs + srow * 256 + (((half * 8 + q) ^ (srow & 7)) << 4));
            v[4 * q] = t4.x * out_scale; v[4 * q + 1] = t4.y * out_scale; v[4 * q + 2] = t4.z * out_scale; v[4 * q + 3] = t4.w * out_scale;
// ... 150 lines not shown
```

### npairloss_b200/csrc/host.cuh

```cuda
#pragma once
#include <cuda.h>
#include <cuda_runtime.h>

#include <cstdarg>
#include <cstdio>
#include <cstring>
#include <string>
#include <vector>

#include "../../include/npair_b200.h"
#include "gemm_wgmma.cuh"
#include "grad_fused.cuh"
#include "kernels.cuh"

namespace npair {

extern thread_local std::string g_create_err;

inline std::string fmt(const char* f, ...) {
  char buf[1024];
  va_list ap; va_start(ap, f); vsnprintf(buf, sizeof(buf), f, ap); va_end(ap);
  return std::string(buf);
}

bool make_tmap_pieces(CUtensorMap* m, const void* base, int cols, int rows, int pieces, long long ld_elems, long long piece_stride_elems,
                      int bk, int box_rows, std::string* err);
bool make_tmap_kcat(CUtensorMap* a, CUtensorMap* b, const uint16_t* A, int rows_a, const uint16_t* B, int rows_b, long long kcat,
                    std::string* err);
bool make_tmap_f32_store(CUtensorMap* m, const void* base, int cols, int rows, long long ld_elems, std::string* err, int box_rows = 32);

constexpr int bk_of(int prec, int epi) {
  if (epi != EPI_OUT) return 64;
  return prec == PREC_BF16 ? 64 : 32;
}

struct GemmKernel { void (*fn)(CUtensorMap, CUtensorMap, CUtensorMap, GemmParams); int threads, smem; };
struct FusedKernel { void (*fn)(CUtensorMap, CUtensorMap, FusedGradParams); int threads, smem; };
template <class K>
cudaError_t allow_smem(const K& k) {
  return k.fn ? cudaFuncSetAttribute(k.fn, cudaFuncAttributeMaxDynamicSharedMemorySize, k.smem) : cudaErrorInvalidValue;
}
GemmKernel gemm_kernel(int prec, int epi);
cudaError_t launch_gemm(int prec, int epi, const CUtensorMap& a, const CUtensorMap& b, const CUtensorMap& sm, const GemmParams& p, int sms, cudaStream_t st);
FusedKernel fused_kernel(int prec);
cudaError_t launch_fused_grad(int prec, const CUtensorMap& b, const CUtensorMap& sm, const FusedGradParams& p, int sms, cudaStream_t st);
cudaError_t launch_simt_gemm(int prec, int epi, const uint16_t* A, long long lda, long long psA, const uint16_t* B, long long ldb,
                             long long psB, int K, const GemmParams& p, cudaStream_t st);
__global__ void splitk_reduce_kernel(const float* __restrict__ part, int splits, long long n, float* __restrict__ out, float beta);

struct SplitK { int splits, kb_per_split; };
inline int split_k_cap(int num_kblocks, int tiles, int sms, int min_kb) {
  int splits = sms / (tiles > 0 ? tiles : 1);
  if (splits > 16) splits = 16;
  if (splits > num_kblocks / min_kb) splits = num_kblocks / min_kb;
  return splits < 1 ? 1 : splits;
}
inline SplitK split_k(int num_kblocks, int tiles, int sms, int min_kb) {
  const int splits = split_k_cap(num_kblocks, tiles, sms, min_kb);
  const int kpb = (num_kblocks + splits - 1) / splits;
  return SplitK{(num_kblocks + kpb - 1) / kpb, kpb};
}

using TileShape = GemmCfg<1, 64, EPI_OUT>;
static_assert(TileShape::BM == FusedCfg<1>::BM && TileShape::BN == FusedCfg<1>::BN, "both GEMM kernels share one tile shape");
inline TileSched tile_sched(int rows, int cols, int num_kblocks, SplitK sk) {
  return TileSched{num_kblocks, (rows + TileShape::BM - 1) / TileShape::BM, (cols + TileShape::BN - 1) / TileShape::BN, nullptr, 0, sk.splits, sk.kb_per_split};
}
inline TileSched tile_sched(int rows, int cols, int num_kblocks) { return tile_sched(rows, cols, num_kblocks, SplitK{1, num_kblocks}); }

inline int grid_for(long long work, int max_blocks) {
  const long long nb = (work + 255) / 256;
  return static_cast<int>(nb < 1 ? 1 : (nb > max_blocks ? max_blocks : nb));
}

inline long long round_up(long long v, long long m) { return (v + m - 1) / m * m; }

inline std::vector<int2> sym_tile_list(int Q, int N) {
  std::vector<int2> tl;
  const TileSched ts = tile_sched(Q, N, 0);
  for (int mb = 0; mb < ts.tiles_m; ++mb)
    for (int nb = mb / 2; nb < ts.tiles_n; ++nb) tl.push_back(make_int2(mb, nb));
  return tl;
}
inline long long sym_tile_count(int Q, int N) {
  const TileSched ts = tile_sched(Q, N, 0);
  long long n = 0;
  for (int mb = 0; mb < ts.tiles_m; ++mb) n += mb / 2 < ts.tiles_n ? ts.tiles_n - mb / 2 : 0;
  return n;
}

inline GemmParams sim_sweep(int epi, int rows, int cols, long long kcat, const float* inv_scale, const int2* sym_tiles, int n_sym_tiles,
                            const RowArrays& ra) {
  GemmParams gp; memset(&gp, 0, sizeof(gp));
  gp.M = rows; gp.Nn = cols;
  gp.ts = tile_sched(rows, cols, static_cast<int>(kcat / 64));
  gp.dev_scale = inv_scale;
  if (epi & EPI_SYM) { gp.ts.tile_list = sym_tiles; gp.ts.num_tiles_list = n_sym_tiles; }
  if (epi & EPI_STATS) {
    gp.st_minw = ra.st_minw; gp.st_maxw = ra.st_maxw; gp.st_maxb = ra.st_maxb; gp.st_maxall = ra.st_maxall; gp.cnt_same = ra.cnt_same;
  }
  return gp;
}

struct Carve {
  char* base;
  size_t bytes = 0;
  template <class T>
  T* take(long long count, size_t align = alignof(T)) {
    bytes = (bytes + align - 1) / align * align;
    T* p = base ? reinterpret_cast<T*>(base + bytes) : nullptr;
    bytes += sizeof(T) * count;
    return p;
  }
};

struct DevMem {
  explicit DevMem(bool allocate = true) : allocate(allocate) {}
  DevMem(const DevMem&) = delete;
  ~DevMem() { release(); }
  template <class T>
  void own(T** p, size_t n, bool zero) {
    if (n == 0 || err != cudaSuccess) return;
    bytes += n;
    if (!allocate) return;
    if ((err = cudaMalloc(p, n)) != cudaSuccess) { *p = nullptr; return; }
    held.push_back(*p);
    if (zero) err = cudaMemset(*p, 0, n);
  }
  template <class F>
  void own_carved(bool zero, F carve) {
    Carve size{nullptr}, cut{nullptr};
    carve(size);
    own(&cut.base, size.bytes, zero);
    carve(cut);
  }
  void release() {
    for (void* q : held) cudaFree(q);
    held.clear(); bytes = 0; err = cudaSuccess;
  }
  const bool allocate;
  size_t bytes = 0;
  cudaError_t err = cudaSuccess;
  std::vector<void*> held;
};

struct StreamOrder {
  StreamOrder() = default;
  StreamOrder(const StreamOrder&) = delete;
  ~StreamOrder() { if (done) cudaEventDestroy(done); }
  cudaError_t create() { return cudaEventCreateWithFlags(&done, cudaEventDisableTiming); }
  void mark(cudaStream_t st) {
    if (!open) return;
    open = false;
    if (cudaEventRecord(done, st) == cudaSuccess) { stream = st; recorded = true; }
  }
  cudaEvent_t done = nullptr;
  cudaStream_t stream = nullptr;
  bool recorded = false;
  bool open = false;
};

inline void carve_stats(Carve& cv, long long rows, RowArrays* ra) {
  ra->st_minw = cv.take<uint32_t>(rows); ra->st_maxw = cv.take<uint32_t>(rows); ra->st_maxb = cv.take<uint32_t>(rows);
  ra->st_maxall = cv.take<uint32_t>(rows); ra->cnt_same = cv.take<int>(rows);
}

#define CUDA_TRY(ctx, call)                                                                              \
  do {                                                                                                   \
    cudaError_t e__ = (call);                                                                            \
    if (e__ != cudaSuccess) {                                                                            \
      (ctx)->err = fmt("%s failed: %s (%s:%d)", #call, cudaGetErrorString(e__), __FILE__, __LINE__);      \
      return NPAIR_E_CUDA;                                                                               \
    }                                                                                                    \
  } while (0)
#define CREATE_TRY(call)                                                                                 \
  do {                                                                                                   \
    cudaError_t e__ = (call);                                                                            \
    if (e__ != cudaSuccess) {                                                                            \
// ... 33 lines not shown
```

### npairloss_b200/csrc/kernels.cu

```cuda
#include <cassert>
#include <cstdlib>
#include "device.cuh"
#include "kernels.cuh"
#include <cuda.h>

#include <cuda_bf16.h>
#include <cuda_fp16.h>
#include <cfloat>

#include "thresholds.cuh"

namespace npair {
unsigned long long g_kernel_launches = 0;


__device__ __forceinline__ float fast_exp_m2(float sv, float m2) {
  float y;
  asm("ex2.approx.ftz.f32 %0, %1;" : "=f"(y) : "f"(fmaf(sv, LOG2E, -m2)));
  return y;
}

template <bool VEC>
__device__ __forceinline__ float4 load4(const float* __restrict__ x, long long q) {
  if (VEC) return __ldg(reinterpret_cast<const float4*>(x) + q);
// ... 69 lines not shown
  for (int b = threadIdx.x; b < static_cast<int>(gridDim.x); b += blockDim.x) { dsum += __ldcg(&partial[b]); mx = fmaxf(mx, __ldcg(&partial[1024 + b])); }
#pragma unroll
  for (int o = 16; o > 0; o >>= 1) { dsum += __shfl_xor_sync(0xffffffffu, dsum, o); mx = fmaxf(mx, __shfl_xor_sync(0xffffffffu, mx, o)); }
  if (l == 0) { s_dsum[w] = dsum; s_max[w] = mx; }
  __syncthreads();
  if (threadIdx.x == 0) {
    dsum = 0.0; mx = 0.f;
    for (int k = 0; k < (blockDim.x >> 5); ++k) { dsum += s_dsum[k]; mx = fmaxf(mx, s_max[k]); }
    bs->asum = static_cast<float>(dsum);
    bs->x_absmax = mx;
    float sc = 1.f, inv = 1.f;
    if (want_scale) { const PreScale ps = pre_scale(mx); sc = ps.scale; inv = ps.inv; }
    bs->x_scale = sc; bs->x_inv_scale = inv;
    bs->err = 0; bs->ticket = 0; bs->ticket2 = 0; bs->ticket0 = 0; bs->ticket3 = 0; bs->sel_active[0] = 0; bs->sel_active[1] = 0;
    bs->cand_n[0] = 0; bs->cand_n[1] = 0;
    bs->n_same = 0; bs->n_diff = 0;
  }
  return true;
}
__global__ void __launch_bounds__(256) prep_reduce_kernel(const float* __restrict__ xl, long long nl, const float* __restrict__ xt, long long ntot,
                                                          float* __restrict__ partial, int want_scale, RowArrays ra, int Q, BlockScalars* bs) {
  prep_reduce_body(xl, nl, xt, ntot, partial, want_scale, ra, Q, bs);
}
void launch_prep_reduce(const float* x_local, long long n_local, const float* x_total, long long n_total, float* partial,
                        int want_scale, RowArrays ra, int Q, BlockScalars* bs, cudaStream_t st) {
  long long nmax = n_local > n_total ? n_local : n_total;
  int nb = static_cast<int>((nmax + 256 * 16 - 1) / (256 * 16));
  if (nb < 1) nb = 1; if (nb > 592) nb = 592;
  prep_reduce_kernel<<<nb, 256, 0, st>>>(x_local, n_local, x_total, n_total, partial, want_scale, ra, Q, bs);
  count_launch();
}
__global__ void __launch_bounds__(256) prep_reduce_memory_kernel(const float* __restrict__ xl, long long nl, const float* __restrict__ xm,
                                                                 long long nm, float* __restrict__ partial, int want_scale, RowArrays ra, int Q,
                                                                 BlockScalars* bs) {
  prep_reduce_body<true>(xl, nl, xm, nm, partial, want_scale, ra, Q, bs);
}
void launch_prep_reduce_memory(const float* x_local, long long n_local, const float* x_mem, long long n_mem, float* partial, int want_scale,
                               RowArrays ra, int Q, BlockScalars* bs, cudaStream_t st) {
  int nb = static_cast<int>((n_local + n_mem + 256 * 16 - 1) / (256 * 16));
  if (nb < 1) nb = 1; if (nb > 592) nb = 592;
  prep_reduce_memory_kernel<<<nb, 256, 0, st>>>(x_local, n_local, x_mem, n_mem, partial, want_scale, ra, Q, bs);
  count_launch();
}

struct SplitArgs {
  const float* x; int N, D;
  uint16_t* Xs; long long ldXs; uint16_t* XsT; long long ldXsT; uint16_t* XlT; long long ldXlT; int row0, Q;
  uint16_t *XcatA, *XcatB; long long Dp;
};
__device__ __forceinline__ void split_load(const SplitArgs& a, int tile_d, int tile_n, float (&v)[8]) {
  const float* __restrict__ x = a.x; const int N = a.N, D = a.D;
  const int t = threadIdx.x, nl = t >> 3, dg = t & 7;
  const int n = tile_n * 32 + nl, d = tile_d * 64 + 8 * dg;
  const bool rowok = n < N;
  if (rowok && d + 7 < D && (D & 3) == 0 && (reinterpret_cast<uintptr_t>(x) & 15) == 0) {
    const float4 a4 = *reinterpret_cast<const float4*>(x + static_cast<long long>(n) * D + d);
    const float4 b4 = *reinterpret_cast<const float4*>(x + static_cast<long long>(n) * D + d + 4);
    v[0] = a4.x; v[1] = a4.y; v[2] = a4.z; v[3] = a4.w; v[4] = b4.x; v[5] = b4.y; v[6] = b4.z; v[7] = b4.w;
  } else {
#pragma unroll
    for (int e = 0; e < 8; ++e) v[e] = (rowok && d + e < D) ? x[static_cast<long long>(n) * D + d + e] : 0.f;
  }
}
template <int PREC>
__device__ __forceinline__ void split_tile(const SplitArgs& a, float sc, int tile_d, int tile_n, const float (&v)[8], int buf) {
  const int N = a.N, D = a.D;
  uint16_t* __restrict__ Xs = a.Xs; const long long ldXs = a.ldXs; uint16_t* __restrict__ XsT = a.XsT; const long long ldXsT = a.ldXsT;
  uint16_t* __restrict__ XlT = a.XlT; const long long ldXlT = a.ldXlT; const int row0 = a.row0, Q = a.Q;
  uint16_t* __restrict__ XcatA = a.XcatA; uint16_t* __restrict__ XcatB = a.XcatB; const long long Dp = a.Dp;
  constexpr int NS = SPLIT_FORMATS[PREC].pieces;
  __shared__ __align__(16) uint16_t tile2[2][NS][64][40];
  uint16_t (*tile)[64][40] = tile2[buf];
  const int n0 = tile_n * 32, d0 = tile_d * 64;
  const int t = threadIdx.x, nl = t >> 3, dg = t & 7;
  const int n = n0 + nl, d = d0 + 8 * dg;
  uint16_t p[8][3];
  uint4 pk[3];
  const bool rowok = n < N;
  split8<PREC>(v, sc, p, pk);
#pragma unroll
  for (int s = 0; s < NS; ++s)
#pragma unroll
    for (int e = 0; e < 8; ++e) tile[s][8 * dg + e][nl] = p[e][s];
  if (rowok && d < Dp) {
    const long long ps = static_cast<long long>(N) * ldXs;
    if (Xs)
#pragma unroll
      for (int s = 0; s < NS; ++s) *reinterpret_cast<uint4*>(Xs + s * ps + static_cast<long long>(n) * ldXs + d) = pk[s];
    if (PREC != PREC_BF16 && XcatA) {
      const long long kcat = mma_passes(NS) * Dp;
      store_kcat_row<PREC>(XcatB + static_cast<long long>(n) * kcat, Dp, d, pk, true);
      if (n >= row0 && n < row0 + Q) store_kcat_row<PREC>(XcatA + static_cast<long long>(n) * kcat, Dp, d, pk, false);
    }
  }
  __syncthreads();
  const int dl = t >> 2, nc = t & 3;
  const int dd = d0 + dl, nn = n0 + 8 * nc;
  if (dd < D && nn < N) {
    const long long pt = static_cast<long long>(D) * ldXsT;
    const long long pl = static_cast<long long>(D) * ldXlT;
#pragma unroll
    for (int s = 0; s < NS; ++s) {
      const uint4 q = *reinterpret_cast<const uint4*>(&tile[s][dl][8 * nc]);
      *reinterpret_cast<uint4*>(XsT + s * pt + static_cast<long long>(dd) * ldXsT + nn) = q;
      if (XlT && nn >= row0 && nn < row0 + Q) {
        if (((nn - row0) & 7) == 0 && nn + 8 <= row0 + Q) *reinterpret_cast<uint4*>(XlT + s * pl + static_cast<long long>(dd) * ldXlT + (nn - row0)) = q;
        else
          for (int e = 0; e < 8; ++e)
            if (nn + e < row0 + Q && nn + e < N) XlT[s * pl + static_cast<long long>(dd) * ldXlT + (nn + e - row0)] = tile[s][dl][8 * nc + e];
      } else if (XlT && nn < row0 && nn + 8 > row0) {
        for (int e = 0; e < 8; ++e)
          if (nn + e >= row0 && nn + e < row0 + Q && nn + e < N) XlT[s * pl + static_cast<long long>(dd) * ldXlT + (nn + e - row0)] = tile[s][dl][8 * nc + e];
      }
    }
  }
}
template <int PREC>
__global__ void __launch_bounds__(256) split_kernel(SplitArgs a, const BlockScalars* __restrict__ bs) {
  float v[8];
  split_load(a, blockIdx.x, blockIdx.y, v);
  split_tile<PREC>(a, (PREC == PREC_FP16X2) ? bs->x_scale : 1.f, blockIdx.x, blockIdx.y, v, 0);
}
__device__ __forceinline__ void split_load_memory(const SplitArgs& a, const float* __restrict__ xm, int tile_d, int tile_n, float (&v)[8]) {
  const int N = a.N, D = a.D;
  const int t = threadIdx.x, nl = t >> 3, dg = t & 7;
  const int n = tile_n * 32 + nl, d = tile_d * 64 + 8 * dg;
  const bool rowok = n < N;
  const float* x = n < a.Q ? a.x + static_cast<long long>(n) * D : xm + static_cast<long long>(n - a.Q) * D;
  if (rowok && d + 7 < D && (reinterpret_cast<uintptr_t>(x) & 15) == 0) {
    const float4 a4 = *reinterpret_cast<const float4*>(x + d);
    const float4 b4 = *reinterpret_cast<const float4*>(x + d + 4);
    v[0] = a4.x; v[1] = a4.y; v[2] = a4.z; v[3] = a4.w; v[4] = b4.x; v[5] = b4.y; v[6] = b4.z; v[7] = b4.w;
  } else {
#pragma unroll
    for (int e = 0; e < 8; ++e) v[e] = (rowok && d + e < D) ? x[d + e] : 0.f;
  }
}
template <int PREC>
__global__ void __launch_bounds__(256) split_memory_kernel(SplitArgs a, const float* __restrict__ xm, const BlockScalars* __restrict__ bs) {
  float v[8];
  split_load_memory(a, xm, blockIdx.x, blockIdx.y, v);
  split_tile<PREC>(a, (PREC == PREC_FP16X2) ? bs->x_scale : 1.f, blockIdx.x, blockIdx.y, v, 0);
}
void launch_split_memory(const float* x, int Q, const float* x_mem, int N, int D, int prec, const BlockScalars* bs, uint16_t* Xs,
                         long long ldXs, uint16_t* XsT, long long ldXsT, uint16_t* XcatA, uint16_t* XcatB, long long Dp, cudaStream_t st) {
  dim3 grid((D + 63) / 64, (N + 31) / 32);
  const SplitArgs a{x, N, D, Xs, ldXs, XsT, ldXsT, nullptr, 0, 0, Q, XcatA, XcatB, Dp};
  with_prec(prec, [&](auto P) { split_memory_kernel<P><<<grid, 256, 0, st>>>(a, x_mem, bs); });
  count_launch();
}
__global__ void memory_rows_kernel(const float* __restrict__ label, int Q, const float* __restrict__ mem_label, int m,
                                   float* __restrict__ lab_total, RowRecord* __restrict__ rec) {
  const int stride = gridDim.x * blockDim.x;
  for (int i = blockIdx.x * blockDim.x + threadIdx.x; i < Q + m; i += stride) {
    if (i < Q) { lab_total[i] = label[i]; continue; }
    const float l = mem_label[i - Q];
    lab_total[i] = l;
    rec[i] = RowRecord::memory(l);
  }
}
void launch_memory_rows(const float* label, int Q, const float* mem_label, int m, float* lab_total, RowRecord* rec, cudaStream_t st) {
  const int blocks = (Q + m + 255) / 256;
  memory_rows_kernel<<<blocks < 1024 ? blocks : 1024, 256, 0, st>>>(label, Q, mem_label, m, lab_total, rec);
  count_launch();
}

void launch_split(const float* x_total, int N, int D, int prec, const BlockScalars* bs, uint16_t* Xs, long long ldXs,
                  uint16_t* XsT, long long ldXsT, uint16_t* XlT, long long ldXlT, int row0_local, int Q,
                  uint16_t* XcatA, uint16_t* XcatB, long long Dp, cudaStream_t st) {
  dim3 grid((D + 63) / 64, (N + 31) / 32);
  const SplitArgs a{x_total, N, D, Xs, ldXs, XsT, ldXsT, XlT, ldXlT, row0_local, Q, XcatA, XcatB, Dp};
  with_prec(prec, [&](auto P) { split_kernel<P><<<grid, 256, 0, st>>>(a, bs); });
  count_launch();
}

// ... 511 lines not shown
```

### npairloss_b200/csrc/kernels.cuh

```cuda
#pragma once
#include <cuda.h>
#include <cuda_runtime.h>
#include <stdint.h>
#include <cmath>
#include <type_traits>

namespace npair {

enum { REGION_GLOBAL = 0, REGION_LOCAL = 1 };
enum { M_HARD = 0, M_EASY = 1, M_RAND = 2, M_RELATIVE_HARD = 3, M_RELATIVE_EASY = 4 };

enum { DERR_EMPTY_LIST = 1, DERR_POS_RANGE = 2 };
enum { DERR_GATHER_SLOT = 4 };
enum { DERR_KMEANS_NO_ARGMAX = 8 };

constexpr float LOG2E = 1.4426950408889634f;

enum { PREC_BF16X3 = 0, PREC_BF16 = 1, PREC_FP16X2 = 2 };
struct SplitFormat {
  int pieces;
  bool bf16;
};
constexpr SplitFormat SPLIT_FORMATS[3] = {{3, true} , {1, true} , {2, false} };
__host__ __device__ constexpr int mma_passes(int pieces) { return pieces * (pieces + 1) / 2; }
template <class F>
inline decltype(auto) with_prec(int prec, F&& f) {
  if (prec == PREC_BF16) return f(std::integral_constant<int, PREC_BF16>());
  if (prec == PREC_FP16X2) return f(std::integral_constant<int, PREC_FP16X2>());
  return f(std::integral_constant<int, PREC_BF16X3>());
}

__host__ __device__ __forceinline__ float ap_sign(int m) { return (m == M_EASY || m == M_RELATIVE_EASY) ? -1.f : 1.f; }
__host__ __device__ __forceinline__ float an_sign(int m) { return (m == M_HARD || m == M_RELATIVE_HARD) ? -1.f : 1.f; }
__device__ __forceinline__ float ap_thr(float t, int m) {
  switch (m) {
    case M_HARD: return nextafterf(t, -INFINITY);
    case M_EASY: return -t;
    case M_RAND: return INFINITY;
    case M_RELATIVE_HARD: return t;
    default: return -t;
  }
}
__device__ __forceinline__ float an_thr(float t, int m) {
  switch (m) {
    case M_HARD: return nextafterf(-t, -INFINITY);
    case M_EASY: return t;
    case M_RAND: return INFINITY;
    case M_RELATIVE_HARD: return -t;
    default: return t;
  }
}

struct RowRecord {
  float4 lo, hi;
  __host__ __device__ static RowRecord make(float m2c, float thr_n, float m2, float label, float thr_p, float cA, float cT) {
    return RowRecord{make_float4(m2c, thr_n, m2, label), make_float4(thr_p, cA, cT, 0.f)};
  }
  __host__ __device__ static RowRecord load(const RowRecord* records, int k) {
    const float4* h = reinterpret_cast<const float4*>(records);
    return RowRecord{h[2 * k], h[2 * k + 1]};
  }
  __host__ __device__ static RowRecord memory(float label) { return make(INFINITY, -INFINITY, INFINITY, label, -INFINITY, 0.f, 0.f); }
  __host__ __device__ float m2c() const { return lo.x; }
  __host__ __device__ float thr_n() const { return lo.y; }
  __host__ __device__ float m2() const { return lo.z; }
  __host__ __device__ float label() const { return lo.w; }
  __host__ __device__ float thr_p() const { return hi.x; }
  __host__ __device__ float cA() const { return hi.y; }
  __host__ __device__ float cT() const { return hi.z; }
};
static_assert(sizeof(RowRecord) == 32, "row records are exchanged as 32 raw bytes");
__host__ __device__ constexpr int weight_scale_log2(int prec) { return prec == PREC_FP16X2 ? 14 : 0; }
constexpr long long ROW_RECORD_FLOATS = sizeof(RowRecord) / sizeof(float);

struct BlockStats {
  unsigned long long n_same;
  float gmin_w, gmax_w, gmax_b;
  int err;
};
static_assert(sizeof(BlockStats) == 24, "block statistics are exchanged as 24 raw bytes");
struct TopSums {
  double loss_sum;
  int hits[3];
  float asum;
  int err;
};
static_assert(sizeof(TopSums) == 32, "tops sums are exchanged as 32 raw bytes");
template <class T>
__host__ __device__ __forceinline__ const T& rank_record(const T* recs, long long stride, int r) {
  return *reinterpret_cast<const T*>(reinterpret_cast<const float*>(recs) + r * stride);
}

struct TopsBlock {
  float tops[5];
  int err;
  unsigned int seq;
};

struct AsyncWords {
  TopsBlock tops;
  unsigned int err;
  float grad_scale;
};

struct BlockScalars {
  unsigned long long n_same, n_diff;
  float gmin_within, gmax_within;
// ... 136 lines not shown
```

### npairloss_b200/csrc/ptx.cuh

```cuda
#pragma once
#include <cuda_runtime.h>
#include <stdint.h>

namespace npair {
namespace ptx {

__device__ __forceinline__ uint32_t smem_u32(const void* p) {
  return static_cast<uint32_t>(__cvta_generic_to_shared(p));
}

__device__ __forceinline__ bool elect_one() {
  uint32_t pred = 0;
  asm volatile(
      "{\n\t.reg .pred P;\n\t"
      "elect.sync _|P, 0xffffffff;\n\t"
      "selp.u32 %0, 1, 0, P;\n\t}\n"
      : "=r"(pred));
  return pred != 0;
}

__device__ __forceinline__ void mbar_init(uint64_t* bar, uint32_t count) {
  asm volatile("mbarrier.init.shared::cta.b64 [%0], %1;" ::"r"(smem_u32(bar)), "r"(count) : "memory");
}
__device__ __forceinline__ void fence_mbar_init() {
  asm volatile("fence.mbarrier_init.release.cluster;" ::: "memory");
}
__device__ __forceinline__ void fence_proxy_async_smem() {
  asm volatile("fence.proxy.async.shared::cta;" ::: "memory");
}
__device__ __forceinline__ void mbar_arrive_expect_tx(uint64_t* bar, uint32_t bytes) {
  asm volatile("mbarrier.arrive.expect_tx.shared::cta.b64 _, [%0], %1;" ::"r"(smem_u32(bar)), "r"(bytes) : "memory");
}
__device__ __forceinline__ void mbar_arrive(uint64_t* bar) {
  asm volatile("mbarrier.arrive.shared::cta.b64 _, [%0];" ::"r"(smem_u32(bar)) : "memory");
}
__device__ __forceinline__ bool mbar_try_wait(uint64_t* bar, uint32_t parity) {
  uint32_t ok;
  asm volatile(
      "{\n\t.reg .pred P;\n\t"
      "mbarrier.try_wait.parity.shared::cta.b64 P, [%1], %2;\n\t"
      "selp.u32 %0, 1, 0, P;\n\t}\n"
      : "=r"(ok)
      : "r"(smem_u32(bar)), "r"(parity)
      : "memory");
  return ok != 0;
}
__device__ __forceinline__ bool mbar_test_wait(uint64_t* bar, uint32_t parity) {
  uint32_t ok;
  asm volatile(
      "{\n\t.reg .pred P;\n\t"
      "mbarrier.test_wait.parity.shared::cta.b64 P, [%1], %2;\n\t"
      "selp.u32 %0, 1, 0, P;\n\t}\n"
      : "=r"(ok)
      : "r"(smem_u32(bar)), "r"(parity)
      : "memory");
  return ok != 0;
}
__device__ __forceinline__ void mbar_wait(uint64_t* bar, uint32_t parity) {
  while (!mbar_try_wait(bar, parity)) {
  }
}

__device__ __forceinline__ void prefetch_tmap(const void* tmap) {
  asm volatile("prefetch.tensormap [%0];" ::"l"(reinterpret_cast<uint64_t>(tmap)) : "memory");
}
__device__ __forceinline__ void tma_load_3d(void* smem_dst, const void* tmap, uint64_t* bar, int32_t c0, int32_t c1, int32_t c2) {
  asm volatile(
      "cp.async.bulk.tensor.3d.shared::cluster.global.mbarrier::complete_tx::bytes [%0], [%1, {%3, %4, %5}], [%2];"
      ::"r"(smem_u32(smem_dst)), "l"(reinterpret_cast<uint64_t>(tmap)), "r"(smem_u32(bar)), "r"(c0), "r"(c1), "r"(c2)
      : "memory");
}
__device__ __forceinline__ void tma_load_2d(void* smem_dst, const void* tmap, uint64_t* bar, int32_t c0, int32_t c1) {
  asm volatile(
      "cp.async.bulk.tensor.2d.shared::cluster.global.mbarrier::complete_tx::bytes [%0], [%1, {%3, %4}], [%2];"
      ::"r"(smem_u32(smem_dst)), "l"(reinterpret_cast<uint64_t>(tmap)), "r"(smem_u32(bar)), "r"(c0), "r"(c1)
      : "memory");
}
__device__ __forceinline__ void tma_store_2d(const void* tmap, const void* smem_src, int32_t c0, int32_t c1) {
  asm volatile("cp.async.bulk.tensor.2d.global.shared::cta.bulk_group [%0, {%2, %3}], [%1];"
               ::"l"(reinterpret_cast<uint64_t>(tmap)), "r"(smem_u32(smem_src)), "r"(c0), "r"(c1)
               : "memory");
}
__device__ __forceinline__ void tma_store_commit() { asm volatile("cp.async.bulk.commit_group;" ::: "memory"); }
template <int N>
__device__ __forceinline__ void tma_store_wait_read() {
  asm volatile("cp.async.bulk.wait_group.read %0;" ::"n"(N) : "memory");
}
template <int N>
__device__ __forceinline__ void tma_store_wait() {
  asm volatile("cp.async.bulk.wait_group %0;" ::"n"(N) : "memory");
}

__device__ __forceinline__ void wgmma_fence() { asm volatile("wgmma.fence.sync.aligned;" ::: "memory"); }
__device__ __forceinline__ void wgmma_commit() { asm volatile("wgmma.commit_group.sync.aligned;" ::: "memory"); }
template <int N>
__device__ __forceinline__ void wgmma_wait() { asm volatile("wgmma.wait_group.sync.aligned %0;" ::"n"(N) : "memory"); }
__device__ __forceinline__ void fence_regs(float (&d)[128]) {
#pragma unroll
  for (int i = 0; i < 128; ++i) asm volatile("" : "+f"(d[i])::"memory");
}

#define NPAIR_ACC_REGS "{%0, %1, %2, %3, %4, %5, %6, %7, %8, %9, %10, %11, %12, %13, %14, %15, %16, %17, %18, %19, %20, %21, %22, %23, %24, %25, %26, %27, %28, %29, %30, %31, %32, %33, %34, %35, %36, %37, %38, %39, %40, %41, %42, %43, %44, %45, %46, %47, %48, %49, %50, %51, %52, %53, %54, %55, %56, %57, %58, %59, %60, %61, %62, %63, %64, %65, %66, %67, %68, %69, %70, %71, %72, %73, %74, %75, %76, %77, %78, %79, %80, %81, %82, %83, %84, %85, %86, %87, %88, %89, %90, %91, %92, %93, %94, %95, %96, %97, %98, %99, %100, %101, %102, %103, %104, %105, %106, %107, %108, %109, %110, %111, %112, %113, %114, %115, %116, %117, %118, %119, %120, %121, %122, %123, %124, %125, %126, %127}"
#define NPAIR_F4(i) "+f"(d[i]), "+f"(d[i + 1]), "+f"(d[i + 2]), "+f"(d[i + 3])
#define NPAIR_F16(i) NPAIR_F4(i), NPAIR_F4(i + 4), NPAIR_F4(i + 8), NPAIR_F4(i + 12)
#define NPAIR_ACC_OUTS(d) NPAIR_F16(0), NPAIR_F16(16), NPAIR_F16(32), NPAIR_F16(48), NPAIR_F16(64), NPAIR_F16(80), NPAIR_F16(96), NPAIR_F16(112)
#define NPAIR_WGMMA(TY, A_AND_B, TAIL, ...)                                                       \
  asm volatile("{\n\t.reg .pred p;\n\tsetp.ne.b32 p, %" TAIL ", 0;\n\t"                              \
               "wgmma.mma_async.sync.aligned.m64n256k16.f32." TY "." TY " " NPAIR_ACC_REGS ", " A_AND_B ";\n\t}\n" \
               : NPAIR_ACC_OUTS(d) : __VA_ARGS__)

template <bool BF16>
__device__ __forceinline__ void wgmma_m64n256k16_ss(float (&d)[128], uint64_t a_desc, uint64_t b_desc, uint32_t scale_d) {
  if (BF16) NPAIR_WGMMA("bf16", "%128, %129, p, 1, 1, 0, 0", "130", "l"(a_desc), "l"(b_desc), "r"(scale_d));
  else NPAIR_WGMMA("f16", "%128, %129, p, 1, 1, 0, 0", "130", "l"(a_desc), "l"(b_desc), "r"(scale_d));
}
template <bool BF16>
__device__ __forceinline__ void wgmma_m64n256k16_rs(float (&d)[128], const uint32_t (&a)[4], uint64_t b_desc, uint32_t scale_d) {
  if (BF16) NPAIR_WGMMA("bf16", "{%128, %129, %130, %131}, %132, p, 1, 1, 0", "133", "r"(a[0]), "r"(a[1]), "r"(a[2]), "r"(a[3]), "l"(b_desc), "r"(scale_d));
  else NPAIR_WGMMA("f16", "{%128, %129, %130, %131}, %132, p, 1, 1, 0", "133", "r"(a[0]), "r"(a[1]), "r"(a[2]), "r"(a[3]), "l"(b_desc), "r"(scale_d));
}
#undef NPAIR_WGMMA
#undef NPAIR_ACC_OUTS
#undef NPAIR_F16
#undef NPAIR_F4
#undef NPAIR_ACC_REGS

__device__ __forceinline__ uint64_t make_kmajor_desc(uint32_t smem_addr, uint32_t sbo_bytes, uint32_t layout_type) {
  uint64_t d = 0;
  d |= static_cast<uint64_t>((smem_addr >> 4) & 0x3FFF);
  d |= static_cast<uint64_t>(1) << 16;
  d |= static_cast<uint64_t>((sbo_bytes >> 4) & 0x3FFF) << 32;
  d |= static_cast<uint64_t>(layout_type & 3) << 62;
  return d;
}

}
}
```

Before: 10.26 million.

## Store split-precision sim operands in piece-interleaved core-matrix layout, drop kcat concatenation

Replaces the k-concatenated operand layout (which duplicated pieces across mma passes, so each operand held mma_passes*Dp elements) with a layout of 8x8 core matrices where all split pieces for a k-block are interleaved. Each k-block is fetched with a single 4D TMA load and consumed by non-swizzled wgmma descriptors. The aim is to cut operand memory and TMA traffic, since only the pieces are stored rather than the duplicated pass combinations. In exchange, the smem layout is unswizzled, which may raise bank conflicts, the BK is smaller, and probe hooks are added under a compile-time macro.

```diff
diff --git a/npairloss_b200/csrc/ctx.cu b/npairloss_b200/csrc/ctx.cu
--- a/npairloss_b200/csrc/ctx.cu
+++ b/npairloss_b200/csrc/ctx.cu
@@ -120,10 +120,26 @@
   return true;
 }
 
-bool make_tmap_kcat(CUtensorMap* a, CUtensorMap* b, const uint16_t* A, int rows_a, const uint16_t* B, int rows_b, long long kcat,
-                    std::string* err) {
-  return make_tmap_pieces(a, A, static_cast<int>(kcat), rows_a, 1, kcat, rows_a * kcat, 64, 128, err) &&
-         make_tmap_pieces(b, B, static_cast<int>(kcat), rows_b, 1, kcat, rows_b * kcat, 64, 256, err);
+static bool make_tmap_sim_side(CUtensorMap* m, const void* base, int rows, SimLayout L, int box_rows, std::string* err) {
+  auto fn = tmap_encode_fn();
+  if (!fn) { *err = "cuTensorMapEncodeTiled entry point not available"; return false; }
+  const cuuint64_t blk = 8ull * L.bk(), kbs = static_cast<cuuint64_t>(L.Dp / L.bk());
+  cuuint64_t dims[4] = {blk, static_cast<cuuint64_t>(L.pieces), kbs, static_cast<cuuint64_t>(L.padded_rows(rows) / 8)};
+  cuuint64_t strides[3] = {blk * 2ull, blk * 2ull * L.pieces, blk * 2ull * L.pieces * kbs};
+  cuuint32_t box[4] = {static_cast<cuuint32_t>(blk), static_cast<cuuint32_t>(L.pieces), 1u, static_cast<cuuint32_t>(box_rows / 8)};
+  cuuint32_t estr[4] = {1u, 1u, 1u, 1u};
+  CUresult r = fn(m, CU_TENSOR_MAP_DATA_TYPE_UINT16, 4, const_cast<void*>(base), dims, strides, box, estr,
+                  CU_TENSOR_MAP_INTERLEAVE_NONE, CU_TENSOR_MAP_SWIZZLE_NONE, CU_TENSOR_MAP_L2_PROMOTION_L2_256B, CU_TENSOR_MAP_FLOAT_OOB_FILL_NONE);
+  if (r != CUDA_SUCCESS) { *err = fmt("cuTensorMapEncodeTiled(sim) failed (%d): rows=%d pieces=%d Dp=%lld", (int)r, rows, L.pieces, L.Dp); return false; }
+  return true;
+}
+
+bool make_tmap_sim(CUtensorMap* a, CUtensorMap* b, const uint16_t* A, int rows_a, const uint16_t* B, int rows_b, SimLayout L,
+                   std::string* err) {
+  if (L.pieces == 1)
+    return make_tmap_pieces(a, A, static_cast<int>(L.Dp), rows_a, 1, L.Dp, rows_a * L.Dp, L.bk(), 128, err) &&
+           make_tmap_pieces(b, B, static_cast<int>(L.Dp), rows_b, 1, L.Dp, rows_b * L.Dp, L.bk(), 256, err);
+  return make_tmap_sim_side(a, A, rows_a, L, 128, err) && make_tmap_sim_side(b, B, rows_b, L, 256, err);
 }
 
 bool make_tmap_f32_store(CUtensorMap* m, const void* base, int cols, int rows, long long ld_elems, std::string* err, int box_rows) {
@@ -215,7 +231,7 @@
 struct Plan {
   int N, nsplit, bk_grad;
   long long Dp, Np, Qp, ldS;
-  long long kcat;
+  SimLayout sim;
   int bwd_mode;
   bool fused_grad;
   bool cat;
@@ -242,7 +258,7 @@
   p.N = static_cast<int>(N);
   p.nsplit = SPLIT_FORMATS[prec].pieces; p.bk_grad = bk_of(prec, EPI_OUT);
   p.Dp = round_up(D, 64); p.Np = round_up(N, 64); p.Qp = round_up(Q, 64); p.ldS = round_up(N, 32);
-  p.kcat = mma_passes(p.nsplit) * p.Dp;
+  p.sim = SimLayout{p.nsplit, p.Dp};
   const int blk_rows = sim_block_rows(cfg);
   p.s_rows = blk_rows ? blk_rows : cfg.Q;
   p.n_blocks = (cfg.Q + p.s_rows - 1) / p.s_rows;
@@ -344,7 +360,7 @@
   m.own(&c->S, f * c->s_rows * c->ldS, true);
   if (!c->cat) m.own(&c->Xs, 2 * ns * N * c->Dp, true);
   m.own(&c->XsT, 2 * ns * D * c->Np, true);
-  if (c->cat) { m.own(&c->XcatA, 2 * Q * c->cfg.world * c->kcat, true); m.own(&c->XcatB, 2 * N * c->kcat, true); }
+  if (c->cat) { m.own(&c->XcatA, 2 * c->sim.elems(Q), true); m.own(&c->XcatB, 2 * c->sim.elems(N), true); }
   if (!c->fused_grad) m.own(&c->H, 2 * ns * Q * c->Np, true);
   if (c->bwd_mode == NPAIR_BWDMODE_REDUCE_SCATTER) { m.own(&c->XlT, 2 * ns * D * c->Qp, true); m.own(&c->HT, 2 * ns * N * c->Qp, true); m.own(&c->OUT2, f * N * D, false); }
   if (c->bwd_mode == NPAIR_BWDMODE_ROW_SCALARS) m.own(&c->rs_total, sizeof(RowRecord) * N, false);
@@ -533,9 +549,9 @@
 
 static bool make_maps(npair_ctx* c, std::string* te) {
   const int Q = c->Q, D = c->D, N = c->N, ns = c->nsplit, bkg = c->bk_grad;
-  const uint16_t* catA = c->cat ? c->XcatA : c->Xs;
-  const uint16_t* catB = c->cat ? c->XcatB : c->Xs;
-  bool ok = make_tmap_kcat(&c->tm_simA, &c->tm_simB, catA +static_cast<long long>(c->rank) * Q * c->kcat, Q, catB, N, c->kcat, te);
+  const uint16_t* simA = c->cat ? c->XcatA : c->Xs + static_cast<long long>(c->rank) * Q * c->Dp;
+  const uint16_t* simB = c->cat ? c->XcatB : c->Xs;
+  bool ok = make_tmap_sim(&c->tm_simA, &c->tm_simB, simA, Q, simB, N, c->sim, te);
   ok = ok && make_tmap_f32_store(&c->tm_S, c->S, N, c->s_rows, c->ldS, te);
   if (c->H) ok = ok && make_tmap_pieces(&c->tm_b1A, c->H, N, Q, ns, c->Np, static_cast<long long>(Q) * c->Np, bkg, 128, te);
   ok = ok && make_tmap_pieces(&c->tm_b1B, c->XsT, N, D, ns, c->Np, static_cast<long long>(D) * c->Np, bkg, 256, te);
@@ -892,7 +908,7 @@
 
 static cudaError_t sim_gemm(npair_ctx* c, int epi, int r0, int rows, cudaStream_t st) {
   const SimRows sim = sim_rows(c, r0, rows);
-  GemmParams gp = sim_sweep(epi, rows, c->N, c->kcat, &c->bs->x_inv_scale, c->sym_tiles, c->n_sym_tiles, c->ra);
+  GemmParams gp = sim_sweep(epi, rows, c->N, c->sim, &c->bs->x_inv_scale, c->sym_tiles, c->n_sym_tiles, c->ra);
   gp.a_row0 = sim.row0; gp.S = c->S; gp.ldS = sim.ldS;
   if (epi & EPI_STATS) {
     gp.lab_rows = sim.lab_rows; gp.lab_cols = sim.lab_cols; gp.self_offset = sim.col0;
diff --git a/npairloss_b200/csrc/device.cuh b/npairloss_b200/csrc/device.cuh
--- a/npairloss_b200/csrc/device.cuh
+++ b/npairloss_b200/csrc/device.cuh
@@ -54,18 +54,11 @@
                        p[4][s] | (static_cast<uint32_t>(p[5][s]) << 16), p[6][s] | (static_cast<uint32_t>(p[7][s]) << 16));
 }
 template <int PREC>
-__device__ __forceinline__ void store_kcat_row(uint16_t* row, long long Dp, int d, const uint4 (&pk)[3], bool side_b) {
-  *reinterpret_cast<uint4*>(row + d) = pk[0];
-  if (PREC == PREC_FP16X2) {
-    *reinterpret_cast<uint4*>(row + Dp + 2 * d) = side_b ? pk[1] : pk[0];
-    *reinterpret_cast<uint4*>(row + Dp + 2 * d + 8) = side_b ? pk[0] : pk[1];
-  } else if (PREC == PREC_BF16X3) {
-    *reinterpret_cast<uint4*>(row + Dp + d) = pk[1];
-    *reinterpret_cast<uint4*>(row + 2 * Dp + 2 * d) = side_b ? pk[1] : pk[0];
-    *reinterpret_cast<uint4*>(row + 2 * Dp + 2 * d + 8) = side_b ? pk[0] : pk[1];
-    *reinterpret_cast<uint4*>(row + 4 * Dp + 2 * d) = side_b ? pk[2] : pk[0];
-    *reinterpret_cast<uint4*>(row + 4 * Dp + 2 * d + 8) = side_b ? pk[0] : pk[2];
-  }
+__device__ __forceinline__ void store_sim_row(uint16_t* base, long long Dp, long long n, int d, const uint4 (&pk)[3], bool side_b) {
+  constexpr int NS = SPLIT_FORMATS[PREC].pieces;
+  const SimLayout L{NS, Dp};
+#pragma unroll
+  for (int s = 0; s < NS; ++s) *reinterpret_cast<uint4*>(base + L.offset(n, d, SimLayout::piece_slot(NS, s, side_b))) = pk[s];
 }
 
 __device__ __forceinline__ void reset_row_stats(const RowArrays& ra, long long i) {
diff --git a/npairloss_b200/csrc/eval.cu b/npairloss_b200/csrc/eval.cu
--- a/npairloss_b200/csrc/eval.cu
+++ b/npairloss_b200/csrc/eval.cu
@@ -17,7 +17,8 @@
 
 struct EvalPlan {
   int max_q, max_g, D, prec;
-  long long Dp, kcat;
+  long long Dp;
+  SimLayout sim;
   int n_sym_tiles;
 };
 
@@ -32,7 +33,7 @@
   EvalPlan p{};
   p.max_q = max_q; p.max_g = max_g; p.D = D; p.prec = prec;
   p.Dp = round_up(D, 64);
-  p.kcat = mma_passes(SPLIT_FORMATS[prec].pieces) * p.Dp;
+  p.sim = SimLayout{SPLIT_FORMATS[prec].pieces, p.Dp};
   const int n = max_q < max_g ? max_q : max_g;
   p.n_sym_tiles = static_cast<int>(sym_tile_count(n, n));
   return p;
@@ -54,9 +55,14 @@
   std::string err;
 };
 
+static long long eval_operand_elems(const EvalPlan& p, long long rows) {
+  const long long kept = mma_passes(p.sim.pieces) * p.Dp * rows, need = p.sim.elems(rows);
+  return kept > need ? kept : need;
+}
+
 static cudaError_t eval_buffers(npair_eval* ev, DevMem& m) {
-  m.own(&ev->catA, 2ull * ev->max_q * ev->kcat, false);
-  m.own(&ev->catB, 2ull * ev->max_g * ev->kcat, false);
+  m.own(&ev->catA, 2ull * eval_operand_elems(*ev, ev->max_q), false);
+  m.own(&ev->catB, 2ull * eval_operand_elems(*ev, ev->max_g), false);
   m.own_carved(true, [ev](Carve& cv) { carve_stats(cv, ev->max_q, &ev->ra); ev->absmax_bits = cv.take<unsigned int>(1); });
   m.own(&ev->bs, sizeof(BlockScalars), true);
   m.own(&ev->sym_tiles, sizeof(int2) * ev->n_sym_tiles, false);
@@ -210,7 +216,7 @@
     }
     epi |= EPI_SYM;
   }
-  GemmParams gp = sim_sweep(epi, nq, ng, ev->kcat, &ev->bs->x_inv_scale, ev->sym_tiles, static_cast<int>(ev->sym_host.size()), ev->ra);
+  GemmParams gp = sim_sweep(epi, nq, ng, ev->sim, &ev->bs->x_inv_scale, ev->sym_tiles, static_cast<int>(ev->sym_host.size()), ev->ra);
   gp.self_offset = self_col;
   if (epi & (EPI_STATS | EPI_GATHER | EPI_BUCKET)) { gp.lab_rows = ql; gp.lab_cols = gl; }
   else { gp.cut = cut; gp.count = count; }
@@ -220,7 +226,7 @@
   }
   CUtensorMap ta, tb;
   std::string te;
-  if (!make_tmap_kcat(&ta, &tb, ev->catA, nq, ev->catB, ng, ev->kcat, &te)) { ev->err = te; return NPAIR_E_CUDA; }
+  if (!make_tmap_sim(&ta, &tb, ev->catA, nq, ev->catB, ng, ev->sim, &te)) { ev->err = te; return NPAIR_E_CUDA; }
   CUDA_TRY(ev, launch_gemm(ev->prec, epi, ta, tb, ta, gp, ev->sms, st));
   return NPAIR_OK;
 }
@@ -308,10 +314,10 @@
   if ((rc = eval_prepare(ev, q, nq, g, ng, absmax, false, st)) != NPAIR_OK) return rc;
   CUtensorMap ta, tb;
   std::string te;
-  if (!make_tmap_kcat(&ta, &tb, ev->catA, nq, ev->catB, ng, ev->kcat, &te)) { ev->err = te; return NPAIR_E_CUDA; }
+  if (!make_tmap_sim(&ta, &tb, ev->catA, nq, ev->catB, ng, ev->sim, &te)) { ev->err = te; return NPAIR_E_CUDA; }
   for (int r0 = 0; r0 < nq; r0 += rows) {
     const int m = nq - r0 < rows ? nq - r0 : rows;
-    GemmParams gp = sim_sweep(EPI_STORE_S, m, ng, ev->kcat, &ev->bs->x_inv_scale, nullptr, 0, ev->ra);
+    GemmParams gp = sim_sweep(EPI_STORE_S, m, ng, ev->sim, &ev->bs->x_inv_scale, nullptr, 0, ev->ra);
     gp.a_row0 = r0; gp.S = blk.S; gp.ldS = blk.ldS;
     CUDA_TRY(ev, launch_gemm(ev->prec, EPI_STORE_S, ta, tb, ta, gp, ev->sms, st));
     launch_knn_select(blk.S, blk.ldS, m, ng, k, r0, static_cast<int>(self_col), gallery_row0, d_sim, d_index, st);
@@ -354,8 +360,8 @@
   if ((rc = eval_prepare(ev, x, C, x, C, -1.f, false, st)) != NPAIR_OK) return rc;
   CUtensorMap ta, tb;
   std::string te;
-  if (!make_tmap_kcat(&ta, &tb, ev->catA, C, ev->catB, C, ev->kcat, &te)) { ev->err = te; return NPAIR_E_CUDA; }
-  GemmParams gp = sim_sweep(EPI_STORE_S, C, C, ev->kcat, &ev->bs->x_inv_scale, nullptr, 0, ev->ra);
+  if (!make_tmap_sim(&ta, &tb, ev->catA, C, ev->catB, C, ev->sim, &te)) { ev->err = te; return NPAIR_E_CUDA; }
+  GemmParams gp = sim_sweep(EPI_STORE_S, C, C, ev->sim, &ev->bs->x_inv_scale, nullptr, 0, ev->ra);
   gp.a_row0 = 0; gp.S = cb.S; gp.ldS = cb.ldS;
   CUDA_TRY(ev, launch_gemm(ev->prec, EPI_STORE_S, ta, tb, ta, gp, ev->sms, st));
   CUDA_TRY(ev, cudaMemcpyAsync(cb.pools, pools, sizeof(int32_t) * nb * P, cudaMemcpyHostToDevice, st));
diff --git a/npairloss_b200/csrc/eval_kernels.cu b/npairloss_b200/csrc/eval_kernels.cu
--- a/npairloss_b200/csrc/eval_kernels.cu
+++ b/npairloss_b200/csrc/eval_kernels.cu
@@ -37,12 +37,21 @@
   if (PREC == PREC_FP16X2) ps = pre_scale(absmax >= 0.f ? absmax : __uint_as_float(*absmax_bits));
   if (blockIdx.x == 0 && threadIdx.x == 0 && !side_b) { bs->x_scale = ps.scale; bs->x_inv_scale = ps.inv; }
   const long long groups = Dp / 8, i = static_cast<long long>(blockIdx.x) * blockDim.x + threadIdx.x;
-  if (i >= rows * groups) return;
-  const long long n = i / groups;
-  const int d = static_cast<int>(i - n * groups) * 8;
+  if (i >= SimLayout{NS, Dp}.padded_rows(rows) * groups) return;
+  long long n;
+  int d;
+  if (NS == 1) {
+    n = i / groups; d = static_cast<int>(i - n * groups) * 8;
+  } else {
+    const long long gd = i >> 3, g = gd / groups;
+    n = g * 8 + (i & 7); d = static_cast<int>(gd - g * groups) * 8;
+  }
   const float* xr = x + n * D;
   float v[8];
-  if (d + 7 < D && (D & 3) == 0 && (reinterpret_cast<uintptr_t>(x) & 15) == 0) {
+  if (n >= rows) {
+#pragma unroll
+    for (int e = 0; e < 8; ++e) v[e] = 0.f;
+  } else if (d + 7 < D && (D & 3) == 0 && (reinterpret_cast<uintptr_t>(x) & 15) == 0) {
     const float4 a4 = __ldg(reinterpret_cast<const float4*>(xr + d)), b4 = __ldg(reinterpret_cast<const float4*>(xr + d + 4));
     v[0] = a4.x; v[1] = a4.y; v[2] = a4.z; v[3] = a4.w; v[4] = b4.x; v[5] = b4.y; v[6] = b4.z; v[7] = b4.w;
   } else {
@@ -52,11 +61,11 @@
   uint16_t p[8][3];
   uint4 pk[3];
   split8<PREC>(v, ps.scale, p, pk);
-  store_kcat_row<PREC>(out + n * (mma_passes(NS) * Dp), Dp, d, pk, side_b);
+  store_sim_row<PREC>(out, Dp, n, d, pk, side_b);
 }
 void launch_eval_split(const float* x, int rows, int D, long long Dp, int prec, int side_b, float absmax, const unsigned int* absmax_bits,
                        BlockScalars* bs, uint16_t* out, cudaStream_t st) {
-  const long long work = static_cast<long long>(rows) * (Dp / 8);
+  const long long work = SimLayout{SPLIT_FORMATS[prec].pieces, Dp}.padded_rows(rows) * (Dp / 8);
   with_prec(prec, [&](auto P) {
     eval_split_kernel<P><<<static_cast<unsigned int>((work + 255) / 256), 256, 0, st>>>(x, rows, D, Dp, side_b, absmax, absmax_bits, bs, out);
   });
diff --git a/npairloss_b200/csrc/gemm.cu b/npairloss_b200/csrc/gemm.cu
--- a/npairloss_b200/csrc/gemm.cu
+++ b/npairloss_b200/csrc/gemm.cu
@@ -16,28 +16,29 @@
   using Cfg = GemmCfg<NSPLIT, BK, EPI>;
   return GemmKernel{split_gemm_kernel<NSPLIT, BF16, EPI, BK>, Cfg::THREADS, Cfg::SMEM_BYTES};
 }
-template <bool BF16>
+template <int NS, bool BF16>
 static GemmKernel sim_gemm_t(int epi) {
+  constexpr int BK = SimLayout::bk_of(NS);
   switch (epi) {
-    case EPI_STORE_S | EPI_STATS: return gemm_t<1, BF16, EPI_STORE_S | EPI_STATS, 64>();
-    case EPI_STORE_S | EPI_STATS | EPI_SYM: return gemm_t<1, BF16, EPI_STORE_S | EPI_STATS | EPI_SYM, 64>();
-    case EPI_STATS: return gemm_t<1, BF16, EPI_STATS, 64>();
-    case EPI_STATS | EPI_SYM: return gemm_t<1, BF16, EPI_STATS | EPI_SYM, 64>();
-    case EPI_STORE_S: return gemm_t<1, BF16, EPI_STORE_S, 64>();
-    case EPI_COUNT: return gemm_t<1, BF16, EPI_COUNT, 64>();
-    case EPI_COUNT | EPI_SYM: return gemm_t<1, BF16, EPI_COUNT | EPI_SYM, 64>();
-    case EPI_GATHER: return gemm_t<1, BF16, EPI_GATHER, 64>();
-    case EPI_GATHER | EPI_SYM: return gemm_t<1, BF16, EPI_GATHER | EPI_SYM, 64>();
-    case EPI_BUCKET: return gemm_t<1, BF16, EPI_BUCKET, 64>();
-    case EPI_BUCKET | EPI_SYM: return gemm_t<1, BF16, EPI_BUCKET | EPI_SYM, 64>();
-    case EPI_ARGMAX: return gemm_t<1, BF16, EPI_ARGMAX, 64>();
+    case EPI_STORE_S | EPI_STATS: return gemm_t<NS, BF16, EPI_STORE_S | EPI_STATS, BK>();
+    case EPI_STORE_S | EPI_STATS | EPI_SYM: return gemm_t<NS, BF16, EPI_STORE_S | EPI_STATS | EPI_SYM, BK>();
+    case EPI_STATS: return gemm_t<NS, BF16, EPI_STATS, BK>();
+    case EPI_STATS | EPI_SYM: return gemm_t<NS, BF16, EPI_STATS | EPI_SYM, BK>();
+    case EPI_STORE_S: return gemm_t<NS, BF16, EPI_STORE_S, BK>();
+    case EPI_COUNT: return gemm_t<NS, BF16, EPI_COUNT, BK>();
+    case EPI_COUNT | EPI_SYM: return gemm_t<NS, BF16, EPI_COUNT | EPI_SYM, BK>();
+    case EPI_GATHER: return gemm_t<NS, BF16, EPI_GATHER, BK>();
+    case EPI_GATHER | EPI_SYM: return gemm_t<NS, BF16, EPI_GATHER | EPI_SYM, BK>();
+    case EPI_BUCKET: return gemm_t<NS, BF16, EPI_BUCKET, BK>();
+    case EPI_BUCKET | EPI_SYM: return gemm_t<NS, BF16, EPI_BUCKET | EPI_SYM, BK>();
+    case EPI_ARGMAX: return gemm_t<NS, BF16, EPI_ARGMAX, BK>();
     default: return GemmKernel{nullptr, 0, 0};
   }
 }
 GemmKernel gemm_kernel(int prec, int epi) {
   return with_prec(prec, [epi](auto P) {
     constexpr SplitFormat f = SPLIT_FORMATS[P];
-    return epi != EPI_OUT ? sim_gemm_t<f.bf16>(epi) : gemm_t<f.pieces, f.bf16, EPI_OUT, bk_of(P, EPI_OUT)>();
+    return epi != EPI_OUT ? sim_gemm_t<f.pieces, f.bf16>(epi) : gemm_t<f.pieces, f.bf16, EPI_OUT, bk_of(P, EPI_OUT)>();
   });
 }
 cudaError_t launch_gemm(int prec, int epi, const CUtensorMap& a, const CUtensorMap& b, const CUtensorMap& sm, const GemmParams& p, int sms, cudaStream_t st) {
diff --git a/npairloss_b200/csrc/gemm_wgmma.cuh b/npairloss_b200/csrc/gemm_wgmma.cuh
--- a/npairloss_b200/csrc/gemm_wgmma.cuh
+++ b/npairloss_b200/csrc/gemm_wgmma.cuh
@@ -9,6 +9,10 @@
 #include "thresholds.cuh"
 
 namespace npair {
+
+#ifndef NPAIR_SIM_PROBE
+#define NPAIR_SIM_PROBE 0
+#endif
 
 enum { EPI_OUT = 1, EPI_STORE_S = 8, EPI_STATS = 16, EPI_SYM = 32, EPI_COUNT = 64, EPI_GATHER = 128, EPI_BUCKET = 256, EPI_ARGMAX = 512 };
 
@@ -68,9 +72,12 @@
 struct GemmCfg {
   static constexpr int BM = 128, BN = 256;
   static constexpr int BK = BK_;
+  static constexpr bool PIECED = EPI != EPI_OUT && NSPLIT > 1;
   static constexpr int ROW_BYTES = BK * 2;
-  static constexpr uint32_t LAYOUT = (ROW_BYTES == 128) ? 1u : 2u;
-  static constexpr uint32_t SBO = 8 * ROW_BYTES;
+  static constexpr uint32_t LAYOUT = PIECED ? 0u : (ROW_BYTES == 128) ? 1u : 2u;
+  static constexpr uint32_t SBO = PIECED ? 8 * NSPLIT * ROW_BYTES : 8 * ROW_BYTES;
+  static constexpr uint32_t CORE = 128;
+  static constexpr uint32_t SLOT = 8 * ROW_BYTES;
   static constexpr int A_PIECE = BM * ROW_BYTES;
   static constexpr int B_PIECE = BN * ROW_BYTES;
   static constexpr int STAGE_BYTES = NSPLIT * (A_PIECE + B_PIECE);
@@ -84,6 +91,7 @@
   static constexpr int SMEM_BYTES = STAGES * STAGE_BYTES + ACC_STAGE_BYTES + STORE_STAGE_BYTES + SMEM_AUX + 1024 ;
   static constexpr int THREADS = 384;
   static_assert(STAGES >= 2 && 16 * STAGES <= 192, "operand ring");
+  static_assert(!PIECED || BK == SimLayout::bk_of(NSPLIT), "the similarity GEMM's K block is its operands'");
 };
 
 template <int STAGES>
@@ -111,6 +119,25 @@
   const int A[6] = {0, 0, 1, 1, 0, 2};
   const int B[6] = {0, 1, 0, 1, 2, 0};
   sa = A[p]; sb = B[p];
+}
+
+template <int NSPLIT, bool BF16, class Cfg>
+__device__ __forceinline__ void sim_kblock_mmas(float (&acc)[128], uint32_t a, uint32_t b) {
+  constexpr int BK = Cfg::BK;
+  const auto slot_a = [](int s) { return SimLayout::piece_slot(NSPLIT, s, false) * Cfg::SLOT; };
+  const auto slot_b = [](int s) { return SimLayout::piece_slot(NSPLIT, s, true) * Cfg::SLOT; };
+#pragma unroll
+  for (int s = 0; s < (NSPLIT == 3 ? 2 : 1); ++s)
+#pragma unroll
+    for (int k = 0; k < BK / 16; ++k)
+      ptx::wgmma_m64n256k16_ss<BF16>(acc, ptx::make_nosw_desc(a + slot_a(s) + 2 * k * Cfg::CORE, Cfg::CORE, Cfg::SBO),
+                                     ptx::make_nosw_desc(b + slot_b(s) + 2 * k * Cfg::CORE, Cfg::CORE, Cfg::SBO), 1u);
+#pragma unroll
+  for (int x = 1; x < NSPLIT; ++x)
+#pragma unroll
+    for (int c = 0; c < BK / 8; ++c)
+      ptx::wgmma_m64n256k16_ss<BF16>(acc, ptx::make_nosw_desc(a + slot_a(0) + c * Cfg::CORE, slot_a(x) - slot_a(0), Cfg::SBO),
+                                     ptx::make_nosw_desc(b + slot_b(x) + c * Cfg::CORE, slot_b(0) - slot_b(x), Cfg::SBO), 1u);
 }
 
 __device__ __forceinline__ bool pair_valid(bool fast, int idx, int limit, int self_idx) { return fast || (idx < limit && idx != self_idx); }
@@ -232,7 +259,8 @@
   using Cfg = GemmCfg<NSPLIT, BK_, EPI>;
   const int worker = static_cast<int>(blockIdx.x), num_workers = static_cast<int>(gridDim.x);
   constexpr int BM = Cfg::BM, BN = Cfg::BN, BK = Cfg::BK, STAGES = Cfg::STAGES;
-  constexpr bool SYM = EPI & EPI_SYM, STORE = EPI & EPI_STORE_S, STATS = EPI & EPI_STATS, COUNT = EPI & EPI_COUNT;
+  constexpr int PROBE = (EPI != EPI_OUT) ? NPAIR_SIM_PROBE : 0;
+  constexpr bool SYM = EPI & EPI_SYM, STORE = EPI & EPI_STORE_S, STATS = (EPI & EPI_STATS) && PROBE != 2, COUNT = EPI & EPI_COUNT;
   constexpr bool GATHER = EPI & EPI_GATHER, BUCKET = EPI & EPI_BUCKET, ARGMAX = EPI & EPI_ARGMAX;
   constexpr bool LABELS = STATS || GATHER || BUCKET;
   static_assert(!ARGMAX || EPI == EPI_ARGMAX, "EPI_ARGMAX is used alone, with full tiles");
@@ -266,12 +294,22 @@
       for (int tile = worker; tile < num_tiles; tile += num_workers) {
         const Tile t = p.ts.at(tile);
         for (int kb = t.kb0; kb < t.kb1; ++kb) {
-          uint64_t* full = ring.produce(Cfg::STAGE_BYTES);
+          uint64_t* full = ring.produce(PROBE == 4 ? 0u : Cfg::STAGE_BYTES);
           uint8_t* st = smem + ring.stage * Cfg::STAGE_BYTES;
-#pragma unroll
-          for (int s = 0; s < NSPLIT; ++s) {
-            ptx::tma_load_3d(st + s * Cfg::A_PIECE, &tmapA, full, kb * BK, t.m_blk * BM + (STORE && !STATS ? p.a_row0 : 0), s);
-            ptx::tma_load_3d(st + NSPLIT * Cfg::A_PIECE + s * Cfg::B_PIECE, &tmapB, full, kb * BK, t.n_blk * BN, s);
+          const bool one = PROBE == 3;
+          const int a_row = t.m_blk * BM + (STORE && !STATS ? p.a_row0 : 0);
+          if constexpr (Cfg::PIECED) {
+            if (PROBE != 4) {
+              ptx::tma_load_4d(st, &tmapA, full, 0, 0, one ? 0 : kb, one ? 0 : a_row / 8);
+              ptx::tma_load_4d(st + NSPLIT * Cfg::A_PIECE, &tmapB, full, 0, 0, one ? 0 : kb, one ? 0 : t.n_blk * BN / 8);
+            }
+            ring.advance();
+            continue;
+          }
+#pragma unroll
+          for (int s = 0; s < NSPLIT && PROBE != 4; ++s) {
+            ptx::tma_load_3d(st + s * Cfg::A_PIECE, &tmapA, full, one ? 0 : kb * BK, one ? 0 : a_row, s);
+            ptx::tma_load_3d(st + NSPLIT * Cfg::A_PIECE + s * Cfg::B_PIECE, &tmapB, full, one ? 0 : kb * BK, one ? 0 : t.n_blk * BN, s);
           }
           ring.advance();
         }
@@ -329,9 +367,12 @@
       int prev = ring.stage;
       for (int kb = t.kb0; kb < t.kb1; ++kb) {
         ring.wait_full();
-        const uint32_t a0 = ptx::smem_u32(smem + ring.stage * Cfg::STAGE_BYTES) + g * 64 * Cfg::ROW_BYTES;
+        const uint32_t a0 = ptx::smem_u32(smem + ring.stage * Cfg::STAGE_BYTES) + g * 8 * Cfg::SBO;
         const uint32_t b0 = ptx::smem_u32(smem + ring.stage * Cfg::STAGE_BYTES) + NSPLIT * Cfg::A_PIECE;
         ptx::wgmma_fence();
+        if constexpr (Cfg::PIECED) {
+          if (PROBE != 1) sim_kblock_mmas<NSPLIT, BF16, Cfg>(acc, a0, b0);
+        } else
 #pragma unroll
         for (int ps = 0; ps < Cfg::NPASS; ++ps) {
           int sa, sb;
@@ -340,7 +381,7 @@
           for (int k4 = 0; k4 < BK / 16; ++k4) {
             const uint64_t ad = ptx::make_kmajor_desc(a0 + sa * Cfg::A_PIECE + k4 * 32, Cfg::SBO, Cfg::LAYOUT);
             const uint64_t bd = ptx::make_kmajor_desc(b0 + sb * Cfg::B_PIECE + k4 * 32, Cfg::SBO, Cfg::LAYOUT);
-            ptx::wgmma_m64n256k16_ss<BF16>(acc, ad, bd, 1u);
+            if (PROBE != 1) ptx::wgmma_m64n256k16_ss<BF16>(acc, ad, bd, 1u);
           }
         }
         ptx::wgmma_commit();
diff --git a/npairloss_b200/csrc/host.cuh b/npairloss_b200/csrc/host.cuh
--- a/npairloss_b200/csrc/host.cuh
+++ b/npairloss_b200/csrc/host.cuh
@@ -25,12 +25,12 @@
 
 bool make_tmap_pieces(CUtensorMap* m, const void* base, int cols, int rows, int pieces, long long ld_elems, long long piece_stride_elems,
                       int bk, int box_rows, std::string* err);
-bool make_tmap_kcat(CUtensorMap* a, CUtensorMap* b, const uint16_t* A, int rows_a, const uint16_t* B, int rows_b, long long kcat,
-                    std::string* err);
+bool make_tmap_sim(CUtensorMap* a, CUtensorMap* b, const uint16_t* A, int rows_a, const uint16_t* B, int rows_b, SimLayout L,
+                   std::string* err);
 bool make_tmap_f32_store(CUtensorMap* m, const void* base, int cols, int rows, long long ld_elems, std::string* err, int box_rows = 32);
 
 constexpr int bk_of(int prec, int epi) {
-  if (epi != EPI_OUT) return 64;
+  if (epi != EPI_OUT) return SimLayout::bk_of(SPLIT_FORMATS[prec].pieces);
   return prec == PREC_BF16 ? 64 : 32;
 }
 
@@ -89,11 +89,11 @@
   return n;
 }
 
-inline GemmParams sim_sweep(int epi, int rows, int cols, long long kcat, const float* inv_scale, const int2* sym_tiles, int n_sym_tiles,
+inline GemmParams sim_sweep(int epi, int rows, int cols, SimLayout L, const float* inv_scale, const int2* sym_tiles, int n_sym_tiles,
                             const RowArrays& ra) {
   GemmParams gp; memset(&gp, 0, sizeof(gp));
   gp.M = rows; gp.Nn = cols;
-  gp.ts = tile_sched(rows, cols, static_cast<int>(kcat / 64));
+  gp.ts = tile_sched(rows, cols, static_cast<int>(L.Dp / L.bk()));
   gp.dev_scale = inv_scale;
   if (epi & EPI_SYM) { gp.ts.tile_list = sym_tiles; gp.ts.num_tiles_list = n_sym_tiles; }
   if (epi & EPI_STATS) {
diff --git a/npairloss_b200/csrc/kernels.cu b/npairloss_b200/csrc/kernels.cu
--- a/npairloss_b200/csrc/kernels.cu
+++ b/npairloss_b200/csrc/kernels.cu
@@ -175,15 +175,19 @@
   for (int s = 0; s < NS; ++s)
 #pragma unroll
     for (int e = 0; e < 8; ++e) tile[s][8 * dg + e][nl] = p[e][s];
-  if (rowok && d < Dp) {
+  if (rowok && d < Dp && Xs) {
     const long long ps = static_cast<long long>(N) * ldXs;
-    if (Xs)
-#pragma unroll
-      for (int s = 0; s < NS; ++s) *reinterpret_cast<uint4*>(Xs + s * ps + static_cast<long long>(n) * ldXs + d) = pk[s];
-    if (PREC != PREC_BF16 && XcatA) {
-      const long long kcat = mma_passes(NS) * Dp;
-      store_kcat_row<PREC>(XcatB + static_cast<long long>(n) * kcat, Dp, d, pk, true);
-      if (n >= row0 && n < row0 + Q) store_kcat_row<PREC>(XcatA + static_cast<long long>(n) * kcat, Dp, d, pk, false);
+#pragma unroll
+    for (int s = 0; s < NS; ++s) *reinterpret_cast<uint4*>(Xs + s * ps + static_cast<long long>(n) * ldXs + d) = pk[s];
+  }
+  if (PREC != PREC_BF16 && XcatA && d < Dp) {
+    const SimLayout L{NS, Dp};
+    if (n < L.padded_rows(N)) store_sim_row<PREC>(XcatB, Dp, n, d, pk, true);
+    if (n >= row0 && n < row0 + L.padded_rows(Q)) {
+      uint4 pa[3];
+#pragma unroll
+      for (int s = 0; s < 3; ++s) pa[s] = n < row0 + Q ? pk[s] : make_uint4(0u, 0u, 0u, 0u);
+      store_sim_row<PREC>(XcatA, Dp, n - row0, d, pa, false);
     }
   }
   __syncthreads();
diff --git a/npairloss_b200/csrc/kernels.cuh b/npairloss_b200/csrc/kernels.cuh
--- a/npairloss_b200/csrc/kernels.cuh
+++ b/npairloss_b200/csrc/kernels.cuh
@@ -23,6 +23,21 @@
 };
 constexpr SplitFormat SPLIT_FORMATS[3] = {{3, true} , {1, true} , {2, false} };
 __host__ __device__ constexpr int mma_passes(int pieces) { return pieces * (pieces + 1) / 2; }
+
+struct SimLayout {
+  int pieces;
+  long long Dp;
+  __host__ __device__ constexpr static int bk_of(int pieces) { return pieces == 1 ? 64 : (pieces == 2 ? 32 : 16); }
+  __host__ __device__ int bk() const { return bk_of(pieces); }
+  __host__ __device__ long long padded_rows(long long rows) const { return pieces == 1 ? rows : (rows + 7) / 8 * 8; }
+  __host__ __device__ long long elems(long long rows) const { return padded_rows(rows) * pieces * Dp; }
+  __host__ __device__ static int piece_slot(int pieces, int s, bool side_b) { return side_b ? (s == 0 ? pieces - 1 : s - 1) : s; }
+  __host__ __device__ long long offset(long long n, long long k, int slot) const {
+    if (pieces == 1) return n * Dp + k;
+    const int bk = bk_of(pieces);
+    return (((n >> 3) * (Dp / bk) + k / bk) * pieces + slot) * 8 * bk + (k % bk) / 8 * 64 + (n & 7) * 8;
+  }
+};
 template <class F>
 inline decltype(auto) with_prec(int prec, F&& f) {
   if (prec == PREC_BF16) return f(std::integral_constant<int, PREC_BF16>());
diff --git a/npairloss_b200/csrc/ptx.cuh b/npairloss_b200/csrc/ptx.cuh
--- a/npairloss_b200/csrc/ptx.cuh
+++ b/npairloss_b200/csrc/ptx.cuh
@@ -70,6 +70,12 @@
       ::"r"(smem_u32(smem_dst)), "l"(reinterpret_cast<uint64_t>(tmap)), "r"(smem_u32(bar)), "r"(c0), "r"(c1), "r"(c2)
       : "memory");
 }
+__device__ __forceinline__ void tma_load_4d(void* smem_dst, const void* tmap, uint64_t* bar, int32_t c0, int32_t c1, int32_t c2, int32_t c3) {
+  asm volatile(
+      "cp.async.bulk.tensor.4d.shared::cluster.global.mbarrier::complete_tx::bytes [%0], [%1, {%3, %4, %5, %6}], [%2];"
+      ::"r"(smem_u32(smem_dst)), "l"(reinterpret_cast<uint64_t>(tmap)), "r"(smem_u32(bar)), "r"(c0), "r"(c1), "r"(c2), "r"(c3)
+      : "memory");
+}
 __device__ __forceinline__ void tma_load_2d(void* smem_dst, const void* tmap, uint64_t* bar, int32_t c0, int32_t c1) {
   asm volatile(
       "cp.async.bulk.tensor.2d.shared::cluster.global.mbarrier::complete_tx::bytes [%0], [%1, {%3, %4}], [%2];"
@@ -133,6 +139,13 @@
   d |= static_cast<uint64_t>(layout_type & 3) << 62;
   return d;
 }
+__device__ __forceinline__ uint64_t make_nosw_desc(uint32_t smem_addr, uint32_t lbo_bytes, uint32_t sbo_bytes) {
+  uint64_t d = 0;
+  d |= static_cast<uint64_t>((smem_addr >> 4) & 0x3FFF);
+  d |= static_cast<uint64_t>((lbo_bytes >> 4) & 0x3FFF) << 16;
+  d |= static_cast<uint64_t>((sbo_bytes >> 4) & 0x3FFF) << 32;
+  return d;
+}
 
 }
 }
```

Result: faster. 10.75 million (median of 6 runs) (+4.8%).
